# Schatten2021/rust-raytracing

Measured on AMD Instinct MI355X. Metric: Mrays/s (primary rays, whole node), 10k-sphere 1080p 64spp, higher is better.
Workload: dtype f64; 1 GPU; C2: 10k random spheres (scene seed 1), 1920x1080, 64 spp; width=1920, height=1080, rays_per_pixel=64, n_objects=10000, partition=single GPU

## Files before the change

### rust-raytracing_amd/__init__.py

```python
import ctypes as C
import math

import numpy as np

from . import abi
from .abi import (RTX_TUNE_NO_TILES, RTX_TUNE_NO_QNODES, RTX_TUNE_NO_PACKETS, RTX_TUNE_WF_PURE, RTX_TUNE_ONE_STAGE,
                  RTX_TUNE_TWO_STAGE, RTX_TUNE_BVH_MEDIAN, RTX_TUNE_TRI_LEAF_SHIFT, RTX_TUNE_THRESH_SHIFT, RTX_TUNE_PK_LDS_STACK, RTX_TUNE_NO_CUT, RTX_TUNE_INLINE_LEAVES, RTX_TUNE_HALVES, RTX_TUNE_NO_HALVES, RTX_TUNE_NO_TILE_LISTS)
from .abi import (OBJECT_DTYPE, RTX_KERNEL_WAVEFRONT, RTX_KERNEL_AUTO, RTX_KERNEL_BVH, RTX_KERNEL_EXACT, RTX_KERNEL_MIXED, RTX_KERNEL_MIXED_VERIFY, RTX_KERNEL_BVH_REGROUP,
                  RTX_PLANE, RTX_SPHERE, RTX_TRIANGLE, RtxError, load_library, RAY_DTYPE, HIT_DTYPE, FEATURE_DTYPE)

__all__ = ["LabKernel", "Vector3", "Material", "Sphere", "Plane", "Triangle", "Object", "Config", "Camera", "Scene",
           "SceneHandle", "RtxError", "device_count", "pack_objects", "OBJECT_DTYPE",
           "RTX_KERNEL_AUTO", "RTX_KERNEL_EXACT", "RTX_KERNEL_MIXED", "RTX_KERNEL_MIXED_VERIFY", "RTX_KERNEL_BVH", "RTX_KERNEL_BVH_REGROUP", "RTX_KERNEL_WAVEFRONT", "debug_host_scene",
           "RAY_DTYPE", "HIT_DTYPE", "FEATURE_DTYPE", "make_rays"]


class Vector3:
    __slots__ = ("x", "y", "z")

    def __init__(self, x=0.0, y=0.0, z=0.0):
        self.x, self.y, self.z = float(x), float(y), float(z)

    @staticmethod
    def zeros():
# ... 338 lines not shown
        sc = _scene_c(self.config, self.camera, packed)
        lib = load_library(self.config.wants_lab())
        abi.check(lib.rtx_any_hits(C.byref(sc), rays.ctypes.data, lim.ctypes.data if lim is not None else None, len(rays),
                                   occ.ctypes.data), lib)
        return occ.astype(bool)

    def multi_hits(self, origins, directions, k, t_max=None):
        rays = make_rays(origins, directions)
        n, k = len(rays), int(k)
        lim = _limits(t_max, n)
        hits = np.zeros((n, max(k, 0)), dtype=HIT_DTYPE)
        counts = np.zeros(n, dtype=np.uint32)
        packed = self.packed()
        sc = _scene_c(self.config, self.camera, packed)
        lib = load_library(self.config.wants_lab())
        abi.check(lib.rtx_multi_hits(C.byref(sc), rays.ctypes.data, lim.ctypes.data if lim is not None else None, n, k, hits.ctypes.data,
                                     counts.ctypes.data), lib)
        return _split_hits(hits) + (counts,)

    def trace_paths(self, origins, directions, ids=None):
        rays = make_rays(origins, directions)
        n = len(rays)
        pid = _path_ids(ids, n)
        rgb = np.zeros((n, 3), dtype=np.float64)
        seg = np.zeros(n, dtype=np.uint32)
        packed = self.packed()
        sc = _scene_c(self.config, self.camera, packed)
        lib = load_library(self.config.wants_lab())
        abi.check(lib.rtx_trace_paths(C.byref(sc), rays.ctypes.data, pid.ctypes.data if pid is not None else None, n, rgb.ctypes.data,
                                      seg.ctypes.data), lib)
        return rgb, seg


    def features(self, width, height):
        width, height = int(width), int(height)
        out = np.zeros((height, width), dtype=FEATURE_DTYPE)
        packed = self.packed()
        sc = _scene_c(self.config, self.camera, packed)
        lib = load_library(self.config.wants_lab())
        abi.check(lib.rtx_pixel_features(C.byref(sc), width, height, out.ctypes.data), lib)
        return _split_features(out)


TILE_LIST_WALK = 0xFFFFFFFF


class SceneHandle:

    def __init__(self, scene, device=0, lab=None):
        self.lab = scene.config.wants_lab() if lab is None else bool(lab)
        self._lib = load_library(self.lab)
        self.device = int(device)
        self.rays_per_pixel = int(scene.config.rays_per_pixel)
        self._h = C.c_void_p()
        packed = scene.packed()
        sc = _scene_c(scene.config, scene.camera, packed)
        self._check(self._lib.rtx_scene_upload(C.byref(sc), self.device, C.byref(self._h)))
        self._n_objects = len(packed)

    def _check(self, status):
        abi.check(status, self._lib)

    def set_config(self, config):
        if config.wants_lab() and not self.lab:
            raise ValueError("this handle lives in the product library; a lab config needs scene.upload(lab=True)")
        c = config.to_c()
        self._check(self._lib.rtx_scene_set_config(self._h, C.byref(c)))
        self.rays_per_pixel = int(config.rays_per_pixel)

    def set_scratch_limit(self, n_bytes):
        self._check(self._lib.rtx_scene_set_scratch_limit(self._h, int(n_bytes)))

    def set_camera(self, camera):
        c = camera.to_c()
        self._check(self._lib.rtx_scene_set_camera(self._h, C.byref(c)))

    def append_objects(self, packed):
        arr = packed if isinstance(packed, np.ndarray) else pack_objects(packed)
        arr = np.ascontiguousarray(arr, dtype=OBJECT_DTYPE)
        self._check(self._lib.rtx_scene_append_objects(self._h, arr.ctypes.data, len(arr)))
        self._n_objects += len(arr)

    def update_objects(self, indices, packed, mode="auto", stream=None):
        arr = packed if isinstance(packed, np.ndarray) else pack_objects(packed)
        arr = np.ascontiguousarray(arr, dtype=OBJECT_DTYPE)
        idx = np.ascontiguousarray(np.asarray(indices, dtype=np.uint64).reshape(-1))
        if len(idx) != len(arr):
            raise ValueError("update_objects: %d indices for %d objects" % (len(idx), len(arr)))
        how = C.c_uint32(0)
        self._check(self._lib.rtx_scene_update_objects(self._h, idx.ctypes.data, arr.ctypes.data, len(arr), _update_mode(mode),
                                                       C.c_void_p(int(stream)) if stream else None, C.byref(how)))
        return UPDATE_HOW[how.value]

    def set_visible(self, indices, visible, stream=None):
        idx = np.ascontiguousarray(np.asarray(indices, dtype=np.uint64).reshape(-1))
        how = C.c_uint32(0)
        self._check(self._lib.rtx_scene_set_visible(self._h, idx.ctypes.data if len(idx) else None, len(idx), int(visible),
                                                    C.c_void_p(int(stream)) if stream else None, C.byref(how)))
        return UPDATE_HOW[how.value]

    def hide(self, indices):
        return self.set_visible(indices, False)

    def show(self, indices):
        return self.set_visible(indices, True)

    def visible(self):
        mask = np.zeros(self._n_objects, dtype=np.uint8)
        self._check(self._lib.rtx_scene_get_visible(self._h, mask.ctypes.data if len(mask) else None))
        return mask.astype(bool)

    def debug_resident_digests(self):
        digests = (C.c_uint64 * 8)()
        self._check(self._lib.rtx_debug_resident_digests(self._h, digests))
        return tuple(int(v) for v in digests)

    def debug_resident_mesh_digests(self):
        digests = (C.c_uint64 * 16)()
        self._check(self._lib.rtx_debug_resident_mesh_digests(self._h, digests))
        return tuple(int(v) for v in digests)

    def debug_paths(self, width, height, row, max_steps):
        spp = self.rays_per_pixel
        steps = np.zeros((int(width), spp, int(max_steps)), dtype=PATH_STEP_DTYPE)
        counts = np.zeros((int(width), spp), dtype=np.uint32)
        self._check(self._lib.rtx_debug_paths(self._h, int(width), int(height), int(row), int(max_steps), steps.ctypes.data, counts.ctypes.data))
        return steps, counts

    def debug_path_bounds(self, origins, directions, objects, best_up, form=0, path_steps=0, want_records=False):
        rays = make_rays(origins, directions)
        n = len(rays)
        obj = np.ascontiguousarray(np.broadcast_to(np.asarray(objects, dtype=np.uint32), (n,)))
        bu = np.ascontiguousarray(np.broadcast_to(np.asarray(best_up, dtype=np.float32), (n,)))
        out = np.zeros((n, 8), dtype=np.uint32)
        extra = bool(want_records) or int(path_steps) > 0
        info = np.zeros(16, dtype=np.float64)
        rec = np.zeros((n, 16), dtype=np.uint32)
        path = np.zeros((n, int(path_steps), 16), dtype=np.uint32)
        self._check(self._lib.rtx_debug_path_bounds(self._h, rays.ctypes.data, obj.ctypes.data, bu.ctypes.data, n, int(form), out.ctypes.data,
                                                    info.ctypes.data if extra else None, rec.ctypes.data if extra else None,
                                                    path.ctypes.data if int(path_steps) > 0 else None, int(path_steps)))
        return (out, info, rec, path) if extra else out

    def debug_tile_lists(self):
        info = np.zeros(8, dtype=np.uint32)
        self._check(self._lib.rtx_debug_tile_lists(self._h, info.ctypes.data, None, None, 0))
        form, tiles_x, n_tiles, cap = (int(v) for v in info[:4])
        count = np.zeros(n_tiles, dtype=np.uint32)
        ent = np.zeros((n_tiles, cap, 12), dtype=np.uint32)
        if form and n_tiles:
            self._check(self._lib.rtx_debug_tile_lists(self._h, info.ctypes.data, count.ctypes.data, ent.ctypes.data, n_tiles))
        obj = ent[:, :, 9].astype(np.int64)
        obj[obj == 0xFFFFFFFF] = -1
        return {"form": form, "tiles_x": tiles_x, "n_tiles": n_tiles, "cap": cap, "count": count, "raw": ent[:, :, :8].copy(),
                "t_lb": np.ascontiguousarray(ent[:, :, 8]).view(np.float32), "object": obj, "is_record": ent[:, :, 10] == 1}

    def debug_sweep_filter(self, origins, directions, objects=None):
        rays = make_rays(origins, directions)
        n = len(rays)
        info = np.zeros(16, dtype=np.float64)
        obj = None if objects is None else np.ascontiguousarray(np.broadcast_to(np.asarray(objects, dtype=np.uint32), (n,)))
        out = np.zeros((n, 4 if obj is None else 24), dtype=np.uint32)
        self._check(self._lib.rtx_debug_sweep_filter(self._h, rays.ctypes.data if n else None, None if obj is None or not n else obj.ctypes.data,
                                                     n, out.ctypes.data if n else None, info.ctypes.data))
        return out, info

    def render_rows(self, width, height, row_begin, row_stride, n_rows, d_out_ptr, stream=None, want_stats=True):
        stats = abi.RtxStats()
        self._check(self._lib.rtx_render_rows(self._h, int(width), int(height), int(row_begin), int(row_stride),
                                            int(n_rows), C.c_void_p(int(d_out_ptr)),
                                            C.c_void_p(int(stream)) if stream else None,
                                            C.byref(stats) if want_stats else None))
        return stats if want_stats else None

    def render_blocks(self, width, height, block_rows, part, n_parts, d_out_ptr, stream=None, want_stats=True):
        stats = abi.RtxStats()
        self._check(self._lib.rtx_render_blocks(self._h, int(width), int(height), int(block_rows), int(part), int(n_parts),
                                              C.c_void_p(int(d_out_ptr)), C.c_void_p(int(stream)) if stream else None,
                                              C.byref(stats) if want_stats else None))
        return stats if want_stats else None

    def render_accumulate(self, width, height, sample_begin, n_samples, d_sum_ptr, d_sum_sq_ptr=None, block_rows=8, part=0, n_parts=1,
                          stream=None, want_stats=True):
        stats = abi.RtxStats()
        self._check(self._lib.rtx_render_blocks_accumulate(self._h, int(width), int(height), int(block_rows), int(part), int(n_parts),
                                                           int(sample_begin), int(n_samples), C.c_void_p(int(d_sum_ptr)) if d_sum_ptr else None,
                                                           C.c_void_p(int(d_sum_sq_ptr)) if d_sum_sq_ptr else None,
                                                           C.c_void_p(int(stream)) if stream else None, C.byref(stats) if want_stats else None))
        return stats if want_stats else None

    def render_refine(self, width, height, sample_begin, n_more, max_samples, threshold, floor, d_sum_ptr, d_sum_sq_ptr, d_extra_ptr, rounds=1,
                      block_rows=8, part=0, n_parts=1, stream=None, want_stats=True, want_result=True):
        stats = abi.RtxStats()
        result = (C.c_uint64 * 3)()
        self._check(self._lib.rtx_render_blocks_refine(self._h, int(width), int(height), int(block_rows), int(part), int(n_parts),
                                                       int(sample_begin), int(n_more), int(max_samples), int(rounds), float(threshold), float(floor),
                                                       C.c_void_p(int(d_sum_ptr)) if d_sum_ptr else None,
                                                       C.c_void_p(int(d_sum_sq_ptr)) if d_sum_sq_ptr else None,
                                                       C.c_void_p(int(d_extra_ptr)) if d_extra_ptr else None,
                                                       result if want_result else None,
                                                       C.c_void_p(int(stream)) if stream else None, C.byref(stats) if want_stats else None))
        return (tuple(int(v) for v in result) if want_result else None), (stats if want_stats else None)

    def trace_samples(self, width, height, d_ids_ptr, n, d_rgb_ptr, d_segments_ptr=None, stream=None, want_stats=True):
        stats = abi.RtxStats()
        self._check(self._lib.rtx_scene_trace_samples(self._h, int(width), int(height), C.c_void_p(int(d_ids_ptr)) if d_ids_ptr else None, int(n),
                                                      C.c_void_p(int(d_rgb_ptr)) if d_rgb_ptr else None,
                                                      C.c_void_p(int(d_segments_ptr)) if d_segments_ptr else None,
                                                      C.c_void_p(int(stream)) if stream else None, C.byref(stats) if want_stats else None))
        return stats if want_stats else None

    def progressive(self, width, height, moments=True):
        return Progressive(self, width, height, moments)

    def closest_hits(self, d_rays_ptr, n, d_hits_ptr, stream=None, want_stats=True):
        stats = abi.RtxStats()
        self._check(self._lib.rtx_scene_closest_hits(self._h, C.c_void_p(int(d_rays_ptr)), int(n), C.c_void_p(int(d_hits_ptr)),
                                                     C.c_void_p(int(stream)) if stream else None, C.byref(stats) if want_stats else None))
        return stats if want_stats else None

    def primary_hits(self, width, height, d_hits_ptr, stream=None, want_stats=True):
        stats = abi.RtxStats()
        self._check(self._lib.rtx_scene_primary_hits(self._h, int(width), int(height), C.c_void_p(int(d_hits_ptr)),
                                                     C.c_void_p(int(stream)) if stream else None, C.byref(stats) if want_stats else None))
        return stats if want_stats else None

    def any_hits(self, d_rays_ptr, d_t_max_ptr, n, d_out_ptr, stream=None, want_stats=True):
        stats = abi.RtxStats()
        self._check(self._lib.rtx_scene_any_hits(self._h, C.c_void_p(int(d_rays_ptr)),
                                                 C.c_void_p(int(d_t_max_ptr)) if d_t_max_ptr else None, int(n), C.c_void_p(int(d_out_ptr)),
                                                 C.c_void_p(int(stream)) if stream else None, C.byref(stats) if want_stats else None))
        return stats if want_stats else None

    def occluded(self, origins, directions, t_max=None):
        import torch
        rays = make_rays(origins, directions)
        n = len(rays)
        lim = _limits(t_max, n)
        dev = torch.device("cuda", self.device)
        d_rays = torch.from_numpy(rays.view(np.uint8)).to(dev)
        d_lim = torch.from_numpy(lim).to(dev) if lim is not None and n else None
        d_out = torch.empty(max(n, 1), dtype=torch.uint8, device=dev)
        torch.cuda.synchronize(dev)
        self.any_hits(d_rays.data_ptr(), d_lim.data_ptr() if d_lim is not None else None, n, d_out.data_ptr(), want_stats=True)
        return d_out[:n].cpu().numpy().astype(bool)

    def multi_hits(self, d_rays_ptr, d_t_max_ptr, n, k, d_hits_ptr, d_counts_ptr=None, stream=None, want_stats=True):
        stats = abi.RtxStats()
        self._check(self._lib.rtx_scene_multi_hits(self._h, C.c_void_p(int(d_rays_ptr)) if d_rays_ptr else None,
                                                   C.c_void_p(int(d_t_max_ptr)) if d_t_max_ptr else None, int(n), int(k),
                                                   C.c_void_p(int(d_hits_ptr)) if d_hits_ptr else None,
                                                   C.c_void_p(int(d_counts_ptr)) if d_counts_ptr else None,
                                                   C.c_void_p(int(stream)) if stream else None, C.byref(stats) if want_stats else None))
        return stats if want_stats else None

    def primary_multi_hits(self, width, height, k, d_hits_ptr, d_counts_ptr=None, stream=None, want_stats=True):
        stats = abi.RtxStats()
        self._check(self._lib.rtx_scene_primary_multi_hits(self._h, int(width), int(height), int(k),
                                                           C.c_void_p(int(d_hits_ptr)) if d_hits_ptr else None,
                                                           C.c_void_p(int(d_counts_ptr)) if d_counts_ptr else None,
                                                           C.c_void_p(int(stream)) if stream else None, C.byref(stats) if want_stats else None))
        return stats if want_stats else None

    def query_all(self, origins, directions, k, t_max=None):
        import torch
        rays = make_rays(origins, directions)
        n, k = len(rays), int(k)
        lim = _limits(t_max, n)
        dev = torch.device("cuda", self.device)
        d_rays = torch.from_numpy(rays.view(np.uint8)).to(dev)
        d_lim = torch.from_numpy(lim).to(dev) if lim is not None and n else None
        d_hits = torch.empty(max(n * k, 1) * HIT_DTYPE.itemsize, dtype=torch.uint8, device=dev)
        d_counts = torch.zeros(max(n, 1), dtype=torch.int32, device=dev)
        torch.cuda.synchronize(dev)
        self.multi_hits(d_rays.data_ptr(), d_lim.data_ptr() if d_lim is not None else None, n, k, d_hits.data_ptr(), d_counts.data_ptr(),
                        want_stats=True)
        hits = d_hits[:n * k * HIT_DTYPE.itemsize].cpu().numpy().view(HIT_DTYPE).reshape(n, k)
        return _split_hits(hits) + (d_counts[:n].cpu().numpy().view(np.uint32),)

    def pick_through(self, width, height, k):
        import torch
        width, height, k = int(width), int(height), int(k)
        n = width * height
        dev = torch.device("cuda", self.device)
        d_hits = torch.empty(max(n * k, 1) * HIT_DTYPE.itemsize, dtype=torch.uint8, device=dev)
        d_counts = torch.zeros(max(n, 1), dtype=torch.int32, device=dev)
        torch.cuda.synchronize(dev)
        self.primary_multi_hits(width, height, k, d_hits.data_ptr(), d_counts.data_ptr(), want_stats=True)
        hits = d_hits[:n * k * HIT_DTYPE.itemsize].cpu().numpy().view(HIT_DTYPE).reshape(height, width, k)
        return _split_hits(hits) + (d_counts[:n].cpu().numpy().view(np.uint32).reshape(height, width),)

    def trace_paths(self, d_rays_ptr, d_ids_ptr, n, d_rgb_ptr, d_segments_ptr=None, stream=None, want_stats=True):
        stats = abi.RtxStats()
        self._check(self._lib.rtx_scene_trace_paths(self._h, C.c_void_p(int(d_rays_ptr)), C.c_void_p(int(d_ids_ptr)) if d_ids_ptr else None,
                                                    int(n), C.c_void_p(int(d_rgb_ptr)),
                                                    C.c_void_p(int(d_segments_ptr)) if d_segments_ptr else None,
                                                    C.c_void_p(int(stream)) if stream else None, C.byref(stats) if want_stats else None))
        return stats if want_stats else None

    def radiance(self, origins, directions, ids=None, samples=1):
        import torch
        rays = make_rays(origins, directions)
        n, samples = len(rays), int(samples)
        if samples < 1:
            raise ValueError("samples >= 1")
        if samples == 1:
            pid = _path_ids(ids, n)
# ... 371 lines not shown
```

### rust-raytracing_amd/build.py

```python
import hashlib
import os
import shutil
import subprocess
from concurrent.futures import ThreadPoolExecutor

HERE = os.path.dirname(os.path.abspath(__file__))
CSRC = os.path.join(HERE, "csrc")
LIB = os.path.join(HERE, "librtx_hip.so")
LAB_LIB = os.path.join(HERE, "librtx_hip_lab.so")
OBJ_DIR = os.path.join(HERE, "build")
SOURCES = ["rtx_kernels.hip", "rtx_bvh_spheres.hip", "rtx_bvh_mesh.hip", "rtx_wavefront.hip", "rtx_query.hip", "rtx_update.hip", "rtx_pack.hip",
           "rtx_api.hip", "rtx_api_update.hip", "rtx_api_debug.hip"]
HEADERS = ["rtx_math.h", "rtx_scene.h", "rtx_bvh.h", "rtx_device.h", "rtx_traverse.h", "rtx_mesh_step.h", "rtx_wavefront.h",
           "rtx_launch.h", "rtx_refit.h", "rtx_pack.h", "rtx_host.h", "rtx_spk_units.h"]
FLAGS = ["--offload-arch=gfx950", "-O3", "-std=c++17", "-fPIC", "-ffp-contract=off",
         "-fno-fast-math", "-Wall", "-Wno-unused-function"]
LAB_FLAGS = ["-DRTX_LAB"]


def hipcc():
    exe = shutil.which("hipcc") or "/opt/rocm/bin/hipcc"
    if not os.path.exists(exe):
        raise RuntimeError("hipcc not found: librtx_hip.so cannot be built (there is no CPU fallback)")
    return exe


def _input_files():
    files = [os.path.join(CSRC, f) for f in HEADERS]
    files.append(os.path.join(HERE, "..", "include", "rtx_hip.h"))
    return files


def _digest(source, flags):
    h = hashlib.sha256()
    h.update(" ".join(flags).encode())
    for f in [os.path.join(CSRC, source)] + _input_files():
        with open(f, "rb") as fh:
            h.update(fh.read())
    return h.hexdigest()[:20]


def build(force=False, extra_flags=(), verbose=False, lib=None, jobs=None, lab=False):
    if lib is None:
        lib = LAB_LIB if lab else LIB
    flags = FLAGS + (LAB_FLAGS if lab else []) + list(extra_flags)
    os.makedirs(OBJ_DIR, exist_ok=True)
    exe = hipcc()
    objs, todo = [], []
    for s in SOURCES:
        obj = os.path.join(OBJ_DIR, "%s.%s.o" % (s[:-4], _digest(s, flags)))
        objs.append(obj)
        if force or not os.path.exists(obj):
            todo.append((s, obj))

    def compile_one(job):
        s, obj = job
        cmd = [exe] + flags + ["-c", os.path.join(CSRC, s), "-o", obj + ".tmp"]
        if verbose:
            print(" ".join(cmd), flush=True)
        subprocess.check_call(cmd)
        os.replace(obj + ".tmp", obj)

    if todo:
        with ThreadPoolExecutor(max_workers=jobs or min(len(todo), max(1, (os.cpu_count() or 2) - 1))) as ex:
            list(ex.map(compile_one, todo))
    stamp = lib + ".objs"
    want = "\n".join(os.path.basename(o) for o in objs) + "\n"
    have = open(stamp).read() if os.path.exists(stamp) else None
    if todo or not os.path.exists(lib) or have != want:
        if os.path.exists(stamp):
            os.remove(stamp)
        cmd = [exe, "--offload-arch=gfx950", "-shared", "-fPIC", "-Wl,-Bsymbolic"] + objs + ["-o", lib + ".tmp"]
        if verbose:
            print(" ".join(cmd), flush=True)
        subprocess.check_call(cmd)
        os.replace(lib + ".tmp", lib)
        with open(stamp, "w") as fh:
            fh.write(want)
    if not extra_flags:
        keep = set()
        for st in os.listdir(HERE):
            if st.endswith(".so.objs") and os.path.exists(os.path.join(HERE, st[:-5])):
                keep.update(open(os.path.join(HERE, st)).read().split())
        for f in os.listdir(OBJ_DIR):
            if f.endswith(".o") and f not in keep:
                os.remove(os.path.join(OBJ_DIR, f))
    return lib


def build_all(force=False, verbose=False):
    return build(force=force, verbose=verbose), build(force=force, verbose=verbose, lab=True)


if __name__ == "__main__":
    import sys
    for path in build_all(force="--force" in sys.argv, verbose=True):
        print(path)
```

### rust-raytracing_amd/csrc/rtx_api.hip

```cpp
#include "rtx_host.h"

#include <cmath>
#include <cstdio>
#include <cstdlib>
#include <cstring>
#include <string>
#include <thread>
#include <vector>

namespace {

bool device_is_gfx950(int dev)
{
    hipDeviceProp_t prop;
    if (hipGetDeviceProperties(&prop, dev) != hipSuccess) return false;
    return std::strncmp(prop.gcnArchName, "gfx950", 6) == 0;
}

constexpr size_t kDefaultScratchBytes = (size_t)24576 << 20;

}

#ifndef RTX_GRABS_PER_WAVE
#define RTX_GRABS_PER_WAVE 16
#endif

constexpr uint64_t kHalvesBelowRays = 0;

constexpr size_t kWorkWords = kQueryRefineWords;

namespace {

template <class T>
int32_t upload_vec(RtxSceneHandle_ *h, const std::vector<T> &v, const T **out)
{
    *out = nullptr;
    if (v.empty()) return RTX_OK;
    void *d = nullptr;
    RTX_HIP_CHECK(hipMalloc(&d, v.size() * sizeof(T)));
    h->scene_allocs.push_back(d);
    RTX_HIP_CHECK(hipMemcpy(d, v.data(), v.size() * sizeof(T), hipMemcpyHostToDevice));
    *out = static_cast<const T *>(d);
    return RTX_OK;
}

void apply_config(RtxSceneHandle_ *h, const RtxConfig &cfg)
{
    h->cfg = cfg;
    h->sv.rays_per_pixel = cfg.rays_per_pixel;
    h->sv.max_bounces = cfg.max_bounces;
    h->sv.focal_length = cfg.focal_length;
    h->sv.focal_offset = cfg.focal_offset;
    h->sv.non_focal_offset = cfg.non_focal_offset;
    h->sv.seed = cfg.seed;
    h->sv.tuning = cfg.tuning;
    h->sv_dirty = true;
}

#ifdef RTX_LAB
constexpr bool kLabBuild = true;
#else
constexpr bool kLabBuild = false;
#endif

int32_t check_config(const RtxConfig &cfg)
{
    if (cfg.kernel > RTX_KERNEL_WAVEFRONT) return fail(RTX_ERR_INVALID_ARGUMENT, "RtxConfig.kernel: unknown kernel id");
    if (cfg.tuning & ~(uint32_t)RTX_TUNE_KNOWN_MASK)
        return fail(RTX_ERR_UNSUPPORTED, "RtxConfig.tuning: a bit include/rtx_hip.h does not name");
    if (!kLabBuild && (cfg.tuning & (uint32_t)RTX_TUNE_LAB_MASK))
        return fail(RTX_ERR_UNSUPPORTED, "RtxConfig.tuning: a RTX_TUNE_LAB_MASK bit selects a kernel that exists in librtx_hip_lab.so only "
                                         "(this is the product library)");
    if (cfg.max_bounces == UINT64_MAX)
        return fail(RTX_ERR_INVALID_ARGUMENT, "RtxConfig.max_bounces + 1 overflows");
    if (cfg.rays_per_pixel > 0xFFFFFFFFull) return fail(RTX_ERR_INVALID_ARGUMENT, "RtxConfig.rays_per_pixel exceeds 2^32-1");
    return RTX_OK;
}

int32_t grow(void **p, size_t *have, size_t want)
{
    if (*have >= want && *p) return RTX_OK;
    if (*p) { RTX_HIP_CHECK(hipFree(*p)); *p = nullptr; *have = 0; }
    if (want == 0) return RTX_OK;
    RTX_HIP_CHECK(hipMalloc(p, want));
    *have = want;
    return RTX_OK;
}

}

RTX_HOST_BEGIN

int usable_device_count()
{
    int n = 0;
    if (hipGetDeviceCount(&n) != hipSuccess) { (void)hipGetLastError(); return 0; }
    int ok = 0;
    for (int d = 0; d < n; ++d) ok += device_is_gfx950(d) ? 1 : 0;
    return ok;
}

void drop_update_tables(RtxSceneHandle_ *h)
{
    auto &b = h->upd;
    for (void *q : { (void *)b.levels, (void *)b.box32, (void *)b.reach, (void *)b.all_levels, (void *)b.tribox32, (void *)b.tri_reach, (void *)b.keep })
        if (q) (void)hipFree(q);
    b.keep = nullptr; b.keep_valid = false;
    b.levels = nullptr; b.box32 = nullptr; b.reach = nullptr; b.valid = false;
    b.all_levels = nullptr; b.tribox32 = nullptr; b.tri_reach = nullptr; b.mesh_valid = false;
}

int32_t upload_packed(RtxSceneHandle_ *h, const PackedScene &p)
{
    const SceneView sv_before = h->sv;
    std::vector<void *> old_allocs;
    old_allocs.swap(h->scene_allocs);
    {
        SceneView sv = p.sv;
        sv.rays_per_pixel = h->sv.rays_per_pixel; sv.max_bounces = h->sv.max_bounces;
        sv.focal_length = h->sv.focal_length; sv.focal_offset = h->sv.focal_offset; sv.non_focal_offset = h->sv.non_focal_offset;
        sv.seed = h->sv.seed; sv.tuning = h->sv.tuning;
        h->sv = sv;
    }
    h->sv.cam_pos = mk(h->cam.position[0], h->cam.position[1], h->cam.position[2]);
    h->sv.to_world_x = mk(h->cam.to_world_space[0], h->cam.to_world_space[1], h->cam.to_world_space[2]);
    h->sv.to_world_y = mk(h->cam.to_world_space[3], h->cam.to_world_space[4], h->cam.to_world_space[5]);
    h->sv.to_world_z = mk(h->cam.to_world_space[6], h->cam.to_world_space[7], h->cam.to_world_space[8]);

    int32_t rc = RTX_OK;
    if (!rc) rc = upload_vec(h, p.bvh4.nodes, &h->sv.bvh_nodes);
    if (!rc) rc = upload_vec(h, p.qnodes, &h->sv.bvh_qnodes);
    if (!rc) rc = upload_vec(h, p.q3nodes, &h->sv.bvh_q3nodes);
    if (!rc) rc = upload_vec(h, p.bvh.prims, &h->sv.bvh_prims);
    if (!rc) rc = upload_vec(h, p.leaf32, &h->sv.bvh_leaf_f32);
    if (!rc) rc = upload_vec(h, p.leaf_cr, &h->sv.bvh_leaf_cr);
    if (!rc) rc = upload_vec(h, p.spheres, &h->sv.spheres);
    if (!rc) rc = upload_vec(h, p.sphere_id, &h->sv.sphere_id);
    if (!rc) rc = upload_vec(h, p.planes, &h->sv.planes);
    if (!rc) rc = upload_vec(h, p.tris, &h->sv.tris);
    if (!rc) rc = upload_vec(h, p.mats, &h->sv.materials);
    if (!rc) rc = upload_vec(h, p.sph32, &h->sv.sphere_f32);
    if (!rc) rc = upload_vec(h, p.tri32, &h->sv.tri_f32);
    if (!rc) rc = upload_vec(h, p.tri_fidx, &h->sv.tri_fidx);
    if (!rc) rc = upload_vec(h, p.tri_geo, &h->sv.tri_geo);
    if (rc) {
        for (void *d : h->scene_allocs) (void)hipFree(d);
        h->scene_allocs.swap(old_allocs);
        h->sv = sv_before;
        return rc;
    }
    for (void *d : old_allocs) (void)hipFree(d);
    h->sv_dirty = true;
    h->refit = make_refit_tables(p);
    drop_update_tables(h);
    return RTX_OK;
}

int32_t check_watchdog(RtxSceneHandle_ *h, bool wait)
{
    if (!h->watchdog_pending) return RTX_OK;
    if (wait) RTX_HIP_CHECK(hipEventSynchronize(h->ev_watchdog));
    else {
        const hipError_t q = hipEventQuery(h->ev_watchdog);
        if (q == hipErrorNotReady) return RTX_OK;
        RTX_HIP_CHECK(q);
    }
    h->watchdog_pending = false;
    if ((h->h_watchdog[0] | h->h_watchdog[1]) != 0ull) {
        const unsigned long long n = h->h_watchdog[0] + h->h_watchdog[1];
        h->h_watchdog[0] = h->h_watchdog[1] = 0ull;
        return fail(RTX_ERR_HIP, "an earlier render on this scene raised its watchdog word (internal error: the sweep kernel's round "
                                 "bound, or a full survivors' queue): " + std::to_string(n) + " event(s); its image is incomplete");
    }
    return RTX_OK;
}

int32_t adopt_stream(RtxSceneHandle_ *h, hipStream_t stream)
{
    if (h->have_last_stream && h->last_stream != stream && h->have_done) RTX_HIP_CHECK(hipStreamWaitEvent(stream, h->ev_done, 0));
    h->last_stream = stream;
    h->have_last_stream = true;
    return RTX_OK;
}

RTX_HOST_END

namespace {

void free_handle(RtxSceneHandle_ *h)
{
    if (!h) return;
    (void)hipSetDevice(h->device);
    for (void *p : h->scene_allocs) (void)hipFree(p);
    drop_update_tables(h);
    if (h->upd.h_entries) (void)hipHostFree(h->upd.h_entries);
    if (h->upd.d_entries) (void)hipFree(h->upd.d_entries);
    if (h->upd.d_status) (void)hipFree(h->upd.d_status);
    if (h->upd.h_status) (void)hipHostFree(h->upd.h_status);
    if (h->samples) (void)hipFree(h->samples);
    if (h->acc) (void)hipFree(h->acc);
    if (h->tables) (void)hipFree(h->tables);
    if (h->h_tables) (void)hipHostFree(h->h_tables);
    if (h->state) (void)hipFree(h->state);
    if (h->wf_state) (void)hipFree(h->wf_state);
    if (h->tile_lists) (void)hipFree(h->tile_lists);
    if (h->counters) (void)hipFree(h->counters);
    if (h->counters_stage1) (void)hipFree(h->counters_stage1);
    if (h->work_counter) (void)hipFree(h->work_counter);
    if (h->d_sv) (void)hipFree(h->d_sv);
    if (h->d_rv) (void)hipFree(h->d_rv);
    {
        auto &b = h->half2;
        if (b.stream) { (void)hipStreamSynchronize(b.stream); (void)hipStreamDestroy(b.stream); }
        for (hipEvent_t e : { b.fork, b.join, b.stage1_done }) if (e) (void)hipEventDestroy(e);
        for (void *q : { (void *)b.counters, (void *)b.counters_stage1, (void *)b.work_counter, (void *)b.d_rv, (void *)b.state, b.queue })
            if (q) (void)hipFree(q);
    }
    if (h->h_watchdog) (void)hipHostFree(h->h_watchdog);
    if (h->ev_watchdog) (void)hipEventDestroy(h->ev_watchdog);
    if (h->ev_done) (void)hipEventDestroy(h->ev_done);
    for (auto &e : h->ev) if (e) (void)hipEventDestroy(e);
    delete h;
}

int32_t check_scene_args(const RtxScene *scene, const char *who)
{
    if (!scene) return fail(RTX_ERR_INVALID_ARGUMENT, std::string(who) + ": null scene");
    if (scene->n_objects && !scene->objects) return fail(RTX_ERR_INVALID_ARGUMENT, std::string(who) + ": objects is null");
    if (scene->n_objects > 0xFFFFFFF0ull) return fail(RTX_ERR_INVALID_ARGUMENT, std::string(who) + ": too many objects");
    return check_config(scene->config);
}

int32_t check_device(int32_t device, const char *who)
{
    int n_dev = 0;
    if (hipGetDeviceCount(&n_dev) != hipSuccess || n_dev == 0) {
        (void)hipGetLastError();
        return fail(RTX_ERR_NO_DEVICE, "no HIP device visible; librtx_hip has no CPU fallback");
    }
    if (device < 0 || device >= n_dev) return fail(RTX_ERR_INVALID_ARGUMENT, std::string(who) + ": bad device index");
    if (!device_is_gfx950(device)) return fail(RTX_ERR_NO_DEVICE, "device is not gfx950 (MI355X); this library targets gfx950 only");
    return RTX_OK;
}

int32_t create_handle(const RtxScene *scene, const PackedScene &p, int32_t device, RtxSceneHandle_ **out)
{
    *out = nullptr;
    RTX_HIP_CHECK(hipSetDevice(device));
    RtxSceneHandle_ *h = new RtxSceneHandle_();
    h->device = device;
    hipDeviceProp_t prop;
    if (hipGetDeviceProperties(&prop, device) != hipSuccess) { free_handle(h); return fail(RTX_ERR_HIP, "hipGetDeviceProperties failed"); }
    h->n_cus = prop.multiProcessorCount;
    h->cam = scene->camera;
    apply_config(h, scene->config);
    if (int32_t irc = upload_packed(h, p)) { free_handle(h); return irc; }
    h->objects.assign(scene->objects, scene->objects + scene->n_objects);

    hipError_t e = hipMalloc((void **)&h->counters, sizeof(Counters) * kCounterShards);
    if (e == hipSuccess) e = hipMalloc((void **)&h->counters_stage1, sizeof(Counters) * kCounterShards);
    if (e == hipSuccess) e = hipMalloc((void **)&h->work_counter, kWorkWords * sizeof(unsigned long long));
    if (e == hipSuccess) e = hipMalloc((void **)&h->d_sv, sizeof(SceneView));
    if (e == hipSuccess) e = hipMalloc((void **)&h->d_rv, sizeof(RowsView));
    if (e == hipSuccess) e = hipHostMalloc((void **)&h->h_watchdog, 2 * sizeof(unsigned long long), hipHostMallocDefault);
    if (e == hipSuccess) { h->h_watchdog[0] = h->h_watchdog[1] = 0ull; e = hipEventCreateWithFlags(&h->ev_watchdog, hipEventDisableTiming); }
    if (e == hipSuccess) e = hipEventCreateWithFlags(&h->ev_done, hipEventDisableTiming);
    for (int k = 0; k < 4 && e == hipSuccess; ++k) e = hipEventCreate(&h->ev[k]);
    if (e != hipSuccess) { free_handle(h); return fail(RTX_ERR_HIP, std::string("scene scratch: ") + hipGetErrorString(e)); }
    *out = h;
    return RTX_OK;
}

size_t scratch_cap(const RtxSceneHandle_ *h, size_t mine_bytes)
{
    size_t cap_bytes = h->scratch_limit ? h->scratch_limit : kDefaultScratchBytes;
    size_t free_b = 0, total_b = 0;
    if (hipMemGetInfo(&free_b, &total_b) == hipSuccess) {
        const size_t avail = (free_b + mine_bytes) / 4 * 3;
        if (cap_bytes > avail) cap_bytes = avail;
    } else (void)hipGetLastError();
    return cap_bytes;
}

struct CounterSums {
    unsigned long long segments = 0, exact = 0, filter = 0, box = 0, mismatches = 0, watchdog = 0;
    void operator+=(const CounterSums &o) { segments += o.segments; exact += o.exact; filter += o.filter; box += o.box; mismatches += o.mismatches; watchdog += o.watchdog; }
    void operator-=(const CounterSums &o) { segments -= o.segments; exact -= o.exact; filter -= o.filter; box -= o.box; mismatches -= o.mismatches; watchdog -= o.watchdog; }
};

CounterSums sum_counters(const Counters (&c)[kCounterShards])
{
    CounterSums s;
    for (int k = 0; k < kCounterShards; ++k) {
        s.segments += c[k].segments; s.exact += c[k].exact_tests; s.filter += c[k].filter_tests;
        if (k >= 2) s.box += c[k].pad_;
    }
    s.mismatches = c[0].pad_; s.watchdog = c[1].pad_;
    return s;
}

int32_t read_counters(const Counters *d_counters, CounterSums &sums)
{
    Counters host[kCounterShards];
    RTX_HIP_CHECK(hipMemcpy(host, d_counters, sizeof host, hipMemcpyDeviceToHost));
    sums = sum_counters(host);
    return RTX_OK;
}

RowsView rows_view(const RtxSceneHandle_ *h, uint32_t width, uint32_t height, uint32_t row_begin, uint32_t row_stride,
                   uint32_t row_block, uint32_t n_rows, uint32_t tiles_x, uint32_t per_sample)
{
    RowsView rv{};
    rv.width = width; rv.height = height;
    rv.row_begin = row_begin; rv.row_stride = row_stride; rv.n_rows = n_rows; rv.row_block = row_block;
    rv.npix = n_rows * width;
    rv.tiles_x = tiles_x;
    rv.div_width = make_fastdiv(width); rv.div_row_block = make_fastdiv(row_block); rv.div_npix = make_fastdiv(rv.npix);
    rv.div_tiles_x = make_fastdiv(tiles_x); rv.div_per_sample = make_fastdiv(per_sample);
    rv.sin_x = h->tables; rv.cos_x = h->tables + width;
    rv.sin_y = h->tables + 2 * (size_t)width; rv.cos_y = rv.sin_y + n_rows;
    return rv;
}

uint32_t grab_size(uint64_t n_rays, int n_cus, uint32_t grabs_per_wave)
{
    const uint64_t per_wave = n_rays / ((uint64_t)n_cus * 16u * grabs_per_wave);
    return (uint32_t)(per_wave >= 512 ? 512 : (per_wave <= 64 ? 64 : (per_wave & ~(uint64_t)63)));
}

int32_t begin_launches(RtxSceneHandle_ *h, hipStream_t stream)
{
    if (h->sv_dirty) {
        RTX_HIP_CHECK(hipMemcpyAsync(h->d_sv, &h->sv, sizeof(SceneView), hipMemcpyHostToDevice, stream));
        h->sv_dirty = false;
    }
    RTX_HIP_CHECK(hipMemsetAsync(h->counters, 0, sizeof(Counters) * kCounterShards, stream));
    return RTX_OK;
}

struct Range { const void *base; size_t bytes; };
bool ranges_overlap(const Range *r, int n)
{
    for (int i = 0; i < n; ++i)
        for (int j = i + 1; j < n; ++j) {
            const uintptr_t a = (uintptr_t)r[i].base, b = (uintptr_t)r[j].base;
            if (a && b && a < b + r[j].bytes && b < a + r[i].bytes) return true;
        }
    return false;
}

}

extern "C" {

int32_t rtx_version(void) { return RTX_HIP_VERSION; }

const char *rtx_last_error(void) { return last_error().c_str(); }

int32_t rtx_device_count(void) { return usable_device_count(); }

int32_t rtx_lab_build(void) { return kLabBuild ? 1 : 0; }

int32_t rtx_camera_new(const double position[3], const double direction[3], double fov, RtxCamera *out)
{
    if (!position || !direction || !out) return fail(RTX_ERR_INVALID_ARGUMENT, "rtx_camera_new: null argument");
    V3 cam_forward = vnorm(mk(direction[0], direction[1], direction[2]));
    V3 cam_right = cross(cam_forward, mk(0., 0., -1.));
    V3 cam_up = cross(cam_forward, cam_right);
    V3 rx = mk(cam_right.x, cam_up.x, cam_forward.x);
    V3 ry = mk(cam_right.y, cam_up.y, cam_forward.y);
    V3 rz = mk(cam_right.z, cam_up.z, cam_forward.z);
    double a = rx.x, b = rx.y, c = rx.z, d = ry.x, e = ry.y, f = ry.z, g = rz.x, hh = rz.y, i = rz.z;
    double sum1 = a * e * i, sum2 = b * f * g, sum3 = c * d * hh;
    double sub1 = g * e * c, sub2 = hh * f * a, sub3 = i * d * b;
    double det = (sum1 + sum2 + sum3) - (sub1 + sub2 + sub3);
    V3 ax = mk(e * i - f * hh, c * hh - b * i, b * f - c * e);
    V3 ay = mk(f * g - d * i, a * i - c * g, c * d - a * f);
    V3 az = mk(d * hh - e * g, b * g - a * hh, a * e - b * d);
    V3 ix = vdivs(ax, det), iy = vdivs(ay, det), iz = vdivs(az, det);
    out->fov = fov;
    for (int k = 0; k < 3; ++k) { out->position[k] = position[k]; out->direction[k] = direction[k]; }
    const V3 w[3] = { rx, ry, rz }, cinv[3] = { ix, iy, iz };
    for (int r = 0; r < 3; ++r) {
        out->to_world_space[3 * r] = w[r].x; out->to_world_space[3 * r + 1] = w[r].y; out->to_world_space[3 * r + 2] = w[r].z;
        out->to_cam_space[3 * r] = cinv[r].x; out->to_cam_space[3 * r + 1] = cinv[r].y; out->to_cam_space[3 * r + 2] = cinv[r].z;
    }
    return RTX_OK;
}

int32_t rtx_scene_upload(const RtxScene *scene, int32_t device, RtxSceneHandle *out)
{
    if (!scene || !out) return fail(RTX_ERR_INVALID_ARGUMENT, "rtx_scene_upload: null argument");
    *out = nullptr;
    if (int32_t rc = check_scene_args(scene, "rtx_scene_upload")) return rc;
    if (int32_t rc = check_device(device, "rtx_scene_upload")) return rc;
    PackedScene p;
    if (int32_t rc = pack_scene(scene, p)) return rc;
    return create_handle(scene, p, device, out);
}

int32_t rtx_scene_free(RtxSceneHandle scene)
{
    if (!scene) return RTX_OK;
    (void)hipSetDevice(scene->device);
    const int32_t rc = check_watchdog(scene, true);
    free_handle(scene);
    return rc;
}

int32_t rtx_scene_set_config(RtxSceneHandle scene, const RtxConfig *config)
{
    if (!scene || !config) return fail(RTX_ERR_INVALID_ARGUMENT, "rtx_scene_set_config: null argument");
    if (int32_t rc = check_config(*config)) return rc;
    if (int32_t rc = check_watchdog(scene, false)) return rc;
    apply_config(scene, *config);
    return RTX_OK;
}

int32_t rtx_scene_set_scratch_limit(RtxSceneHandle scene, uint64_t bytes)
{
    if (!scene) return fail(RTX_ERR_INVALID_ARGUMENT, "rtx_scene_set_scratch_limit: null scene");
    scene->scratch_limit = (size_t)bytes;
    return RTX_OK;
}

int32_t rtx_scene_set_camera(RtxSceneHandle scene, const RtxCamera *camera)
{
    if (!scene || !camera) return fail(RTX_ERR_INVALID_ARGUMENT, "rtx_scene_set_camera: null argument");
    if (int32_t rc = check_watchdog(scene, false)) return rc;
    scene->cam = *camera;
    scene->sv.cam_pos = mk(camera->position[0], camera->position[1], camera->position[2]);
    scene->sv.to_world_x = mk(camera->to_world_space[0], camera->to_world_space[1], camera->to_world_space[2]);
    scene->sv.to_world_y = mk(camera->to_world_space[3], camera->to_world_space[4], camera->to_world_space[5]);
    scene->sv.to_world_z = mk(camera->to_world_space[6], camera->to_world_space[7], camera->to_world_space[8]);
    scene->sv_dirty = true;
    return RTX_OK;
}

}

static uint32_t blocks_row_count(uint32_t height, uint32_t block, uint32_t part, uint32_t n_parts)
{
    if (block == 0 || n_parts == 0 || part >= n_parts) return 0;
    const uint64_t n_blocks = ((uint64_t)height + block - 1) / block;
    if (part >= n_blocks) return 0;
    const uint64_t mine = (n_blocks - part + n_parts - 1) / n_parts;
    uint64_t rows = mine * block;
    const uint64_t last = part + (mine - 1) * (uint64_t)n_parts;
    if (last == n_blocks - 1) rows -= n_blocks * block - height;
    return (uint32_t)rows;
}

static int32_t ensure_tables(RtxSceneHandle_ *h, uint32_t width, uint32_t height, uint32_t row_begin, uint32_t row_stride,
                             uint32_t row_block, uint32_t n_rows, hipStream_t stream)
{
    const size_t tdbl = 2 * (size_t)width + 2 * (size_t)n_rows;
    const bool t_same = h->t_valid && h->t_w == width && h->t_h == height && h->t_rb == row_begin &&
                        h->t_rs == row_stride && h->t_blk == row_block && h->t_nr == n_rows && h->t_fov == h->cam.fov;
    if (!t_same) {
        if (h->have_done) RTX_HIP_CHECK(hipEventSynchronize(h->ev_done));
        if (h->h_tables_doubles < tdbl) {
            if (h->h_tables) RTX_HIP_CHECK(hipHostFree(h->h_tables));
            h->h_tables = nullptr; h->h_tables_doubles = 0;
            RTX_HIP_CHECK(hipHostMalloc((void **)&h->h_tables, tdbl * sizeof(double), hipHostMallocDefault));
            h->h_tables_doubles = tdbl;
        }
        {
            size_t have = h->tables_doubles * sizeof(double);
            if (int32_t rc = grow((void **)&h->tables, &have, tdbl * sizeof(double))) return rc;
            h->tables_doubles = have / sizeof(double);
        }
        const double fov = h->cam.fov;
        const double vertical_fov = (double)height / (double)width * fov;
        double *sx = h->h_tables, *cx = sx + width, *sy = cx + width, *cy = sy + n_rows;
        for (uint32_t x = 0; x < width; ++x) {
            double u = (double)x / (double)width;
            double angle_x = fov * (u - 0.5);
            ::sincos(angle_x, &sx[x], &cx[x]);
        }
        for (uint32_t k = 0; k < n_rows; ++k) {
            const uint32_t kb = k / row_block;
            double v = (double)(row_begin + kb * row_stride + (k - kb * row_block)) / (double)height;
            double angle_y = vertical_fov * (v - 0.5);
            ::sincos(angle_y, &sy[k], &cy[k]);
        }
        RTX_HIP_CHECK(hipMemcpyAsync(h->tables, h->h_tables, tdbl * sizeof(double), hipMemcpyHostToDevice, stream));
        h->t_w = width; h->t_h = height; h->t_rb = row_begin; h->t_rs = row_stride; h->t_blk = row_block; h->t_nr = n_rows;
        h->t_fov = fov; h->t_valid = true;
    }
    return RTX_OK;
}

namespace {

struct BandPlan {
    uint32_t kernel = RTX_KERNEL_AUTO;
    bool tiled = false; uint32_t tiles_x = 0;
    uint64_t per_sample64 = 0, batch = 0;
    uint64_t tile_list_bytes = 0;
    bool spheres_kernel = false, mesh_kernel = false, spheres_two_stage = false;
    bool halves = false;
};
struct BandRun { float trace_ms = 0.f, resolve_ms = 0.f, stage1_ms = 0.f; CounterSums stage1; uint32_t launches = 0; };

uint32_t choose_kernel(const SceneView &sv, const RtxConfig &cfg, uint32_t npix, uint64_t spp)
{
    const uint64_t outside_tree = ((sv.bvh_flags & 1u) ? 0u : sv.n_spheres) + (uint64_t)(sv.n_tri_filter - sv.n_tri_tree);
    uint32_t kernel = cfg.kernel;
    const bool want_tiles = (cfg.tuning & RTX_TUNE_NO_TILES) == 0u;
    if (kernel == RTX_KERNEL_AUTO) {
        if (sv.n_bvh_nodes != 0 && outside_tree <= 64) {
            const bool mesh = (sv.bvh_flags & 2u) != 0u && sv.n_tri_tree >= 1024u;
            kernel = mesh ? RTX_KERNEL_BVH_REGROUP : RTX_KERNEL_BVH;
            if (mesh && (uint64_t)npix * spp >= (1ull << 20) && want_tiles && wavefront_mesh_supported(sv, true))
                kernel = RTX_KERNEL_WAVEFRONT;
        } else {
            kernel = RTX_KERNEL_MIXED;
        }
    }

    if (kernel == RTX_KERNEL_BVH || kernel == RTX_KERNEL_BVH_REGROUP || kernel == RTX_KERNEL_WAVEFRONT) {
        const bool sphere_tree = sv.n_bvh_nodes != 0 && (sv.bvh_flags & 19u) == 17u;
        const bool tri_tree = sv.n_bvh_nodes != 0 && (sv.bvh_flags & 2u) != 0u;
        if (sphere_tree) kernel = RTX_KERNEL_BVH;
        else if (!tri_tree) kernel = RTX_KERNEL_MIXED;
        else if (kernel == RTX_KERNEL_BVH) kernel = RTX_KERNEL_BVH_REGROUP;
    }
    if (kernel == RTX_KERNEL_WAVEFRONT && !wavefront_mesh_supported(sv, want_tiles)) kernel = RTX_KERNEL_BVH_REGROUP;
    return kernel;
}

int32_t plan_batch(const RtxSceneHandle_ *h, BandPlan &plan, uint32_t width, uint32_t n_rows, uint64_t spp)
{
    const uint32_t kernel = plan.kernel, tuning = h->cfg.tuning;
    const bool want_tiles = (tuning & RTX_TUNE_NO_TILES) == 0u;
    plan.tiled = (kernel == RTX_KERNEL_BVH || kernel == RTX_KERNEL_BVH_REGROUP || kernel == RTX_KERNEL_WAVEFRONT) && want_tiles;
    plan.tiles_x = plan.tiled ? (width + 7u) / 8u : 0u;
    const uint64_t per_sample64 = plan.tiled ? (uint64_t)plan.tiles_x * ((n_rows + 7u) / 8u) * 64u : (uint64_t)n_rows * width;
    if (per_sample64 > 0xFFFFFFF0ull) return fail(RTX_ERR_INVALID_ARGUMENT, "rtx_render_rows: more than 2^32 ray slots per sample");
    plan.per_sample64 = per_sample64;
    plan.batch = spp;
    const bool sph2 = kernel == RTX_KERNEL_BVH && (h->sv.bvh_flags & 2u) == 0u && h->sv.n_bvh_nodes != 0;
    const uint64_t per_ray = 4 * sizeof(double) + (kernel == RTX_KERNEL_WAVEFRONT ? wavefront_state_bytes(1u << 20, 1) >> 20 : 0) +
                             (sph2 ? 64 + 5 : 0);
    const size_t cap_bytes = scratch_cap(h, h->samples_bytes + h->wf_bytes + h->tile_lists_bytes);
    if ((tuning & RTX_TUNE_NO_TILE_LISTS) == 0u && plan.tiled) {
        if (sph2) plan.tile_list_bytes = bvh_spheres_tile_list_bytes(per_sample64);
        else if (kernel == RTX_KERNEL_WAVEFRONT) plan.tile_list_bytes = wavefront_tile_list_bytes(per_sample64);
        if (plan.tile_list_bytes > cap_bytes / 4) plan.tile_list_bytes = 0;
    }
    const uint64_t fixed = plan.tile_list_bytes +
                           (sph2 ? (uint64_t)bvh_spheres_queue_bytes(0, h->n_cus) + bvh_spheres_spill_bytes(h->sv, h->n_cus) : 0) +
                           (kernel == RTX_KERNEL_WAVEFRONT ? (uint64_t)wavefront_state_bytes(0, 1) + wavefront_spill_bytes(h->sv, h->n_cus) : 0) +
                           (kernel == RTX_KERNEL_MIXED || kernel == RTX_KERNEL_MIXED_VERIFY ? (uint64_t)mixed_state_bytes(h->n_cus) : 0);
    const uint64_t room = cap_bytes > fixed ? cap_bytes - fixed : 0;
    const uint64_t fit = room * 8 / (per_sample64 * (per_ray * 8 + 1));
    const uint64_t fit32 = 0xFFFFFFF0ull / per_sample64;
    if (plan.batch > fit) plan.batch = fit ? fit : 1;
    if (plan.batch > fit32) plan.batch = fit32;
    return RTX_OK;
}

void plan_forms(const RtxSceneHandle_ *h, BandPlan &plan, uint64_t spp, bool may_halve)
{
    const SceneView &sv = h->sv;
    const uint32_t kernel = plan.kernel, tuning = h->cfg.tuning;
    plan.spheres_kernel = kernel == RTX_KERNEL_BVH && (sv.bvh_flags & 2u) == 0u && sv.n_bvh_nodes != 0;
    plan.mesh_kernel = kernel == RTX_KERNEL_BVH_REGROUP && (sv.bvh_flags & 2u) != 0u;
    plan.spheres_two_stage = plan.spheres_kernel && h->cfg.max_bounces > 0 && (tuning & RTX_TUNE_ONE_STAGE) == 0u &&
                             (plan.batch * plan.per_sample64 >= (1ull << 20) || (tuning & RTX_TUNE_TWO_STAGE) != 0u) &&
                             bvh_spheres_two_stage_ok(sv, plan.tiled);
    const bool halves_can = may_halve && plan.spheres_two_stage && plan.batch == spp && spp >= 2;
    plan.halves = halves_can && (tuning & RTX_TUNE_NO_HALVES) == 0u &&
                  ((tuning & RTX_TUNE_HALVES) != 0u || plan.per_sample64 * spp <= kHalvesBelowRays);
}

int32_t grow_scratch(RtxSceneHandle_ *h, const BandPlan &plan, uint32_t npix, uint64_t spp, bool own_acc)
{
    const uint32_t kernel = plan.kernel;
    const uint64_t batch_rays = plan.batch * plan.per_sample64;
    if (spp > 0)
        if (int32_t rc = grow((void **)&h->samples, &h->samples_bytes,
                              (size_t)(batch_rays * 4 * sizeof(double)) + nonzero_mask_bytes(batch_rays))) return rc;
    if (own_acc && plan.batch < spp)
        if (int32_t rc = grow((void **)&h->acc, &h->acc_bytes, (size_t)npix * 3 * sizeof(double))) return rc;
    if (kernel == RTX_KERNEL_BVH || kernel == RTX_KERNEL_BVH_REGROUP) {
        if (!plan.spheres_kernel && !plan.mesh_kernel) return fail(RTX_ERR_HIP, "internal: no tree kernel for this scene");
        const size_t need = plan.spheres_kernel ? bvh_spheres_spill_bytes(h->sv, h->n_cus) : bvh_mesh_spill_bytes(h->sv, h->n_cus);
        if (int32_t rc = grow((void **)&h->state, &h->state_bytes, need)) return rc;
    }
    if (kernel == RTX_KERNEL_MIXED || kernel == RTX_KERNEL_MIXED_VERIFY)
        if (int32_t rc = grow((void **)&h->state, &h->state_bytes, mixed_state_bytes(h->n_cus))) return rc;
    if (plan.spheres_two_stage) {
        if (int32_t rc = grow(&h->wf_state, &h->wf_bytes, bvh_spheres_queue_bytes(batch_rays, h->n_cus))) return rc;
        if (plan.tile_list_bytes != 0)
            if (int32_t rc = grow(&h->tile_lists, &h->tile_lists_bytes, (size_t)plan.tile_list_bytes)) return rc;
    }
    if (kernel == RTX_KERNEL_WAVEFRONT) {
        if (int32_t rc = grow((void **)&h->state, &h->state_bytes, wavefront_spill_bytes(h->sv, h->n_cus))) return rc;
        if (int32_t rc = grow(&h->wf_state, &h->wf_bytes, wavefront_state_bytes(batch_rays, wavefront_levels(h->sv)))) return rc;
        if (plan.tile_list_bytes != 0)
            if (int32_t rc = grow(&h->tile_lists, &h->tile_lists_bytes, (size_t)plan.tile_list_bytes)) return rc;
    }
    return RTX_OK;
}

uint32_t sphere_flags(uint32_t tuning)
{
    return (tuning & RTX_TUNE_NO_PACKETS) ? 1u : 0u;
}

int32_t launch_halves(RtxSceneHandle_ *h, const BandPlan &plan, RowsView rv, double *d_out_rgb, hipStream_t stream, bool stats,
                      BandRun &run)
{
    const uint64_t spp = h->cfg.rays_per_pixel, per_sample64 = plan.per_sample64;
    auto &b = h->half2;
    if (!b.stream) {
        int least = 0, greatest = 0;
        RTX_HIP_CHECK(hipDeviceGetStreamPriorityRange(&least, &greatest));
        RTX_HIP_CHECK(hipStreamCreateWithPriority(&b.stream, hipStreamNonBlocking, least));
        RTX_HIP_CHECK(hipEventCreateWithFlags(&b.fork, hipEventDisableTiming));
        RTX_HIP_CHECK(hipEventCreateWithFlags(&b.join, hipEventDisableTiming));
        RTX_HIP_CHECK(hipEventCreate(&b.stage1_done));
        RTX_HIP_CHECK(hipMalloc((void **)&b.counters, sizeof(Counters) * kCounterShards));
        RTX_HIP_CHECK(hipMalloc((void **)&b.counters_stage1, sizeof(Counters) * kCounterShards));
        RTX_HIP_CHECK(hipMalloc((void **)&b.work_counter, sizeof(unsigned long long)));
        RTX_HIP_CHECK(hipMalloc((void **)&b.d_rv, sizeof(RowsView)));
    }
    const uint64_t ns[2] = { (spp + 1) / 2, spp / 2 };
    if (int32_t rc = grow((void **)&b.state, &b.state_bytes, bvh_spheres_spill_bytes(h->sv, h->n_cus))) return rc;
    if (int32_t rc = grow(&b.queue, &b.queue_bytes, bvh_spheres_queue_bytes(ns[1] * per_sample64, h->n_cus))) return rc;
    struct Join {
        RtxSceneHandle_ *h; hipStream_t main; bool forked = false;
        ~Join() {
            if (!forked) return;
            if (hipEventRecord(h->half2.join, h->half2.stream) != hipSuccess || hipStreamWaitEvent(main, h->half2.join, 0) != hipSuccess) {
                (void)hipGetLastError(); (void)hipStreamSynchronize(h->half2.stream);
            }
        }
    } join{h, stream};
    RTX_HIP_CHECK(hipMemsetAsync(b.counters, 0, sizeof(Counters) * kCounterShards, stream));
    RTX_HIP_CHECK(hipMemsetAsync(rv.nonzero, 0, nonzero_mask_bytes(per_sample64 * spp), stream));
    if (stats) RTX_HIP_CHECK(hipEventRecord(h->ev[0], stream));
    RTX_HIP_CHECK(hipEventRecord(b.fork, stream));
    RTX_HIP_CHECK(hipStreamWaitEvent(b.stream, b.fork, 0));
    join.forked = true;
    for (int k = 0; k < 2; ++k) {
        RowsView r = rv;
        r.sample_begin = k == 0 ? 0u : (uint32_t)ns[0];
        r.n_samples = (uint32_t)ns[k];
        r.n_rays = per_sample64 * ns[k];
        r.nonzero_base = k == 0 ? 0 : per_sample64 * ns[0];
        r.grab = grab_size(r.n_rays, h->n_cus, RTX_GRABS_PER_WAVE / 2);
        hipStream_t st = k == 0 ? stream : b.stream;
        RTX_HIP_CHECK(hipMemcpyAsync(k == 0 ? h->d_rv : b.d_rv, &r, sizeof(RowsView), hipMemcpyHostToDevice, st));
        RTX_HIP_CHECK(hipMemsetAsync(k == 0 ? h->work_counter : b.work_counter, 0, sizeof(unsigned long long), st));
        RTX_HIP_CHECK(launch_trace_bvh_spheres(h->d_sv, h->sv, k == 0 ? h->d_rv : b.d_rv, r,
                                               h->samples + (k == 0 ? 0 : (size_t)(per_sample64 * ns[0]) * 4), k == 0 ? h->counters : b.counters,
                                               k == 0 ? h->work_counter : b.work_counter, reinterpret_cast<uint32_t *>(k == 0 ? h->state : b.state),
                                               h->n_cus, k == 0 ? h->wf_state : b.queue, sphere_flags(h->cfg.tuning), st,
                                               stats ? (k == 0 ? h->counters_stage1 : b.counters_stage1) : nullptr,
                                               stats ? (k == 0 ? h->ev[3] : b.stage1_done) : nullptr,
                                               nullptr, false));
    }
    RTX_HIP_CHECK(hipEventRecord(b.join, b.stream));
    RTX_HIP_CHECK(hipStreamWaitEvent(stream, b.join, 0));
    join.forked = false;
    run.launches = 1;
    if (stats) RTX_HIP_CHECK(hipEventRecord(h->ev[1], stream));
    rv.sample_begin = 0; rv.n_samples = (uint32_t)spp; rv.n_rays = per_sample64 * spp;
    RTX_HIP_CHECK(launch_resolve(h->samples, h->acc, d_out_rgb, rv, (uint32_t)per_sample64, spp, true, true, stream));
    if (stats) {
        RTX_HIP_CHECK(hipEventRecord(h->ev[2], stream));
        RTX_HIP_CHECK(hipEventSynchronize(h->ev[2]));
        RTX_HIP_CHECK(hipEventElapsedTime(&run.trace_ms, h->ev[0], h->ev[1]));
        RTX_HIP_CHECK(hipEventElapsedTime(&run.resolve_ms, h->ev[1], h->ev[2]));
        float c0 = 0.f, c1 = 0.f;
        RTX_HIP_CHECK(hipEventElapsedTime(&c0, h->ev[0], h->ev[3]));
        RTX_HIP_CHECK(hipEventElapsedTime(&c1, h->ev[0], b.stage1_done));
        run.stage1_ms = c0 > c1 ? c0 : c1;
        for (const Counters *snap : { h->counters_stage1, b.counters_stage1 }) {
            CounterSums s1;
            if (int32_t rc = read_counters(snap, s1)) return rc;
            run.stage1 += s1;
        }
    }
    return RTX_OK;
}

int32_t launch_batch(RtxSceneHandle_ *h, const BandPlan &plan, const RowsView &rv, bool first_batch, hipStream_t stream, bool stats)
{
    const uint32_t kernel = plan.kernel, tuning = h->cfg.tuning;
    uint32_t *const state = reinterpret_cast<uint32_t *>(h->state);
    if (kernel != RTX_KERNEL_EXACT && kernel != RTX_KERNEL_WAVEFRONT)
        RTX_HIP_CHECK(hipMemsetAsync(h->work_counter, 0, sizeof(unsigned long long), stream));
    if (kernel == RTX_KERNEL_EXACT) {
        RTX_HIP_CHECK(launch_trace_exact(h->d_sv, h->d_rv, rv, h->samples, h->counters, stream));
#ifdef RTX_LAB
        if (h->transcript)
            RTX_HIP_CHECK(launch_trace_transcript(h->d_sv, h->d_rv, rv, h->transcript, h->transcript_counts, h->transcript_steps, stream));
#endif
    } else if (kernel == RTX_KERNEL_WAVEFRONT) {
        RTX_HIP_CHECK(launch_trace_wavefront(h->d_sv, h->sv, h->d_rv, rv, h->samples, h->wf_state, h->counters, state, h->n_cus, stream,
                                             plan.tile_list_bytes != 0 ? h->tile_lists : nullptr, first_batch));
    } else if (kernel == RTX_KERNEL_BVH_REGROUP) {
        RTX_HIP_CHECK(launch_trace_bvh_mesh(h->d_sv, h->sv, h->d_rv, rv, h->samples, h->counters, h->work_counter, state, h->n_cus, stream));
    } else if (kernel == RTX_KERNEL_BVH) {
        const bool two = plan.spheres_two_stage;
        RTX_HIP_CHECK(launch_trace_bvh_spheres(h->d_sv, h->sv, h->d_rv, rv, h->samples, h->counters, h->work_counter, state, h->n_cus,
                                               two ? h->wf_state : nullptr, sphere_flags(tuning), stream,
                                               stats && two ? h->counters_stage1 : nullptr, stats && two ? h->ev[3] : nullptr,
                                               two && plan.tile_list_bytes != 0 ? h->tile_lists : nullptr, first_batch));
    } else {
        RTX_HIP_CHECK(launch_trace_mixed(h->d_sv, h->sv, h->d_rv, rv, h->samples, h->state, h->counters, h->work_counter, h->n_cus,
                                         kernel == RTX_KERNEL_MIXED_VERIFY, stream));
    }
    return RTX_OK;
}

int32_t launch_batches(RtxSceneHandle_ *h, const BandPlan &plan, RowsView rv, const SampleRange &sr, double *d_out_rgb, hipStream_t stream,
                       bool stats, BandRun &run)
{
    const uint64_t spp = sr.n;
    const bool accumulate = sr.sum != nullptr;
    CounterSums before;
    for (uint64_t s0 = 0; s0 < spp; s0 += plan.batch) {
        const uint64_t ns = (spp - s0 < plan.batch) ? spp - s0 : plan.batch;
        rv.sample_begin = (uint32_t)(sr.begin + s0); rv.n_samples = (uint32_t)ns;
        rv.n_rays = plan.per_sample64 * ns;
        rv.grab = grab_size(rv.n_rays, h->n_cus, RTX_GRABS_PER_WAVE);
        RTX_HIP_CHECK(hipMemcpyAsync(h->d_rv, &rv, sizeof(RowsView), hipMemcpyHostToDevice, stream));
        RTX_HIP_CHECK(hipMemsetAsync(rv.nonzero, 0, nonzero_mask_bytes(rv.n_rays), stream));
        if (stats) RTX_HIP_CHECK(hipEventRecord(h->ev[0], stream));
        if (int32_t rc = launch_batch(h, plan, rv, s0 == 0, stream, stats)) return rc;
        ++run.launches;
        if (stats) RTX_HIP_CHECK(hipEventRecord(h->ev[1], stream));
        if (accumulate)
            RTX_HIP_CHECK(launch_resolve(h->samples, sr.sum, nullptr, rv, (uint32_t)plan.per_sample64, spp, false, false, stream, sr.sum_sq));
        else
            RTX_HIP_CHECK(launch_resolve(h->samples, h->acc, d_out_rgb, rv, (uint32_t)plan.per_sample64, spp, s0 == 0, s0 + ns == spp, stream));
        if (!stats) continue;
        RTX_HIP_CHECK(hipEventRecord(h->ev[2], stream));
        RTX_HIP_CHECK(hipEventSynchronize(h->ev[2]));
        float a = 0.f, b = 0.f;
        RTX_HIP_CHECK(hipEventElapsedTime(&a, h->ev[0], h->ev[1]));
        RTX_HIP_CHECK(hipEventElapsedTime(&b, h->ev[1], h->ev[2]));
        run.trace_ms += a; run.resolve_ms += b;
        if (plan.spheres_two_stage) {
            float c = 0.f;
            RTX_HIP_CHECK(hipEventElapsedTime(&c, h->ev[0], h->ev[3]));
            run.stage1_ms += c;
            CounterSums snapshot, now;
            if (int32_t rc = read_counters(h->counters_stage1, snapshot)) return rc;
            if (int32_t rc = read_counters(h->counters, now)) return rc;
            run.stage1 += snapshot; run.stage1 -= before;
            before = now;
        }
    }
    return RTX_OK;
}

int32_t finish_stats(RtxSceneHandle_ *h, const BandPlan &plan, const BandRun &run, uint64_t primary_rays, hipStream_t stream, RtxStats *stats)
{
    if (plan.kernel == RTX_KERNEL_MIXED || plan.kernel == RTX_KERNEL_MIXED_VERIFY || plan.spheres_two_stage) {
        if (h->watchdog_pending) RTX_HIP_CHECK(hipEventSynchronize(h->ev_watchdog));
        if (int32_t rc = check_watchdog(h, false)) return rc;
        RTX_HIP_CHECK(hipMemcpyAsync(h->h_watchdog, &h->counters[1].pad_, sizeof(unsigned long long), hipMemcpyDeviceToHost, stream));
        if (plan.halves) RTX_HIP_CHECK(hipMemcpyAsync(h->h_watchdog + 1, &h->half2.counters[1].pad_, sizeof(unsigned long long), hipMemcpyDeviceToHost, stream));
        RTX_HIP_CHECK(hipEventRecord(h->ev_watchdog, stream));
        h->watchdog_pending = true;
    }
    if (!stats) return RTX_OK;
    RTX_HIP_CHECK(hipStreamSynchronize(stream));
    CounterSums c;
    if (int32_t rc = read_counters(h->counters, c)) return rc;
    if (plan.halves) {
        CounterSums more;
        if (int32_t rc = read_counters(h->half2.counters, more)) return rc;
        c += more;
    }
    stats->segments = c.segments; stats->exact_tests = c.exact; stats->filter_tests = c.filter; stats->box_tests = c.box;
    stats->filter_mismatches = c.mismatches;
    if (c.watchdog != 0) {
        h->watchdog_pending = false; h->h_watchdog[0] = h->h_watchdog[1] = 0ull;
        return fail(RTX_ERR_HIP, "trace kernel raised its watchdog word (internal error: round bound / full survivors' queue): " +
                                     std::to_string(c.watchdog) + " event(s)");
    }
    stats->primary_rays = primary_rays;
    stats->trace_ms = run.trace_ms; stats->resolve_ms = run.resolve_ms; stats->stage1_ms = run.stage1_ms;
    stats->trace_launches = run.launches;
    stats->kernel = plan.kernel;
    stats->stage1_box_tests = run.stage1.box; stats->stage1_filter_tests = run.stage1.filter; stats->stage1_exact_tests = run.stage1.exact;
    return RTX_OK;
}

}

RTX_HOST_BEGIN

int32_t render_band(RtxSceneHandle h, uint32_t width, uint32_t height, uint32_t row_begin, uint32_t row_stride,
                    uint32_t row_block, uint32_t n_rows, double *d_out_rgb, void *stream_, RtxStats *stats,
                    const SampleRange *accumulate)
{
    hipStream_t stream = static_cast<hipStream_t>(stream_);
    if (stats) std::memset(stats, 0, sizeof *stats);
    if (n_rows == 0 || width == 0) return RTX_OK;
    if (!accumulate && !d_out_rgb) return fail(RTX_ERR_INVALID_ARGUMENT, "rtx_render_rows: null output");
    if ((uint64_t)n_rows * width > 0xFFFFFFF0ull) return fail(RTX_ERR_INVALID_ARGUMENT, "rtx_render_rows: more than 2^32 pixels per call");
    if (accumulate) {
        if ((uint64_t)n_rows * width >= 0xFFFFFFF0ull)
            return fail(RTX_ERR_INVALID_ARGUMENT, "rtx_render_blocks_accumulate: 2^32 - 16 pixels per call or more");
        const size_t bytes = (size_t)n_rows * width * 3 * sizeof(double);
        const Range r[2] = { { accumulate->sum, bytes }, { accumulate->sum_sq, bytes } };
        if (ranges_overlap(r, 2)) return fail(RTX_ERR_INVALID_ARGUMENT, "rtx_render_blocks_accumulate: d_sum and d_sum_sq overlap");
    }
    RTX_HIP_CHECK(hipSetDevice(h->device));
    if (int32_t rc = check_watchdog(h, false)) return rc;
    if (int32_t rc = adopt_stream(h, stream)) return rc;
    DoneGuard done_guard{h, stream};

    const uint32_t npix = n_rows * width;
    SampleRange sr;
    if (accumulate) sr = *accumulate; else sr.n = h->cfg.rays_per_pixel;
    const uint64_t spp = sr.n;
    if (accumulate && h->sv.n_objects == 0) {
        if (stats) {
            RTX_HIP_CHECK(hipStreamSynchronize(stream));
            stats->primary_rays = (uint64_t)npix * spp;
            stats->kernel = h->cfg.kernel;
        }
        return RTX_OK;
    }
    if (h->sv.n_objects == 0 && spp > 0) {
        RTX_HIP_CHECK(hipMemsetAsync(d_out_rgb, 0, (size_t)npix * 3 * sizeof(double), stream));
        if (stats) {
            RTX_HIP_CHECK(hipStreamSynchronize(stream));
            stats->primary_rays = (uint64_t)npix * spp;
            stats->kernel = h->cfg.kernel;
        }
        return RTX_OK;
    }
    BandPlan plan;
    plan.kernel = choose_kernel(h->sv, h->cfg, npix, spp);
    if (int32_t rc = plan_batch(h, plan, width, n_rows, spp)) return rc;
    plan_forms(h, plan, spp, accumulate == nullptr);
#ifdef RTX_LAB
    h->tl_form = 0;
    if (plan.tile_list_bytes != 0 && spp > 0 && !plan.halves) {
        const bool no_packets = (h->cfg.tuning & RTX_TUNE_NO_PACKETS) != 0u;
        if (plan.kernel == RTX_KERNEL_WAVEFRONT) h->tl_form = (no_packets && (h->sv.bvh_flags & 4u) != 0u) ? 0u : 2u;
        else if (plan.kernel == RTX_KERNEL_BVH && plan.spheres_two_stage) h->tl_form = no_packets ? 0u : 1u;
    }
    h->tl_tiles_x = plan.tiles_x;
    h->tl_tiles = (uint32_t)(plan.per_sample64 >> 6);
#endif
    if (int32_t rc = ensure_tables(h, width, height, row_begin, row_stride, row_block, n_rows, stream)) return rc;
    if (int32_t rc = grow_scratch(h, plan, npix, spp, accumulate == nullptr)) return rc;

    RowsView rv = rows_view(h, width, height, row_begin, row_stride, row_block, n_rows, plan.tiles_x, (uint32_t)plan.per_sample64);
    rv.nonzero = spp > 0 ? reinterpret_cast<uint32_t *>(h->samples + (size_t)(plan.batch * plan.per_sample64) * 4) : nullptr;
    if (int32_t rc = begin_launches(h, stream)) return rc;
    BandRun run;
    if (spp == 0) {
        rv.n_samples = 0; rv.n_rays = 0; rv.tiles_x = 0;
        RTX_HIP_CHECK(launch_resolve(nullptr, nullptr, d_out_rgb, rv, npix, 0, true, true, stream));
    } else if (plan.halves) {
        if (int32_t rc = launch_halves(h, plan, rv, d_out_rgb, stream, stats != nullptr, run)) return rc;
    } else {
        if (int32_t rc = launch_batches(h, plan, rv, sr, d_out_rgb, stream, stats != nullptr, run)) return rc;
    }
    return finish_stats(h, plan, run, (uint64_t)npix * spp, stream, stats);
}

RTX_HOST_END

namespace {

struct QueryRequest {
    uint32_t mode = kQueryClosest;
    uint32_t width = 0, height = 0;
    uint32_t row_begin = 0, row_stride = 1, row_block = 1, n_rows = 0;
    uint64_t n = 0;
    const RtxRay *rays = nullptr;
    RtxHit *hits = nullptr;
    uint8_t *occluded = nullptr; const double *t_max = nullptr;
    double *rgb = nullptr;
    const uint64_t *ids = nullptr; uint32_t *segments = nullptr;
    RtxPixelFeatures *features = nullptr;
    double *sum = nullptr, *sum_sq = nullptr; uint32_t *extra = nullptr;
    double threshold = 0.0, floor = 0.0;
    uint32_t sample_begin = 0, n_more = 0, max_samples = 0, rounds = 0;
    uint64_t *result = nullptr;
    uint32_t k = 0; uint32_t *counts = nullptr;
};

}

static int32_t query_run(RtxSceneHandle_ *h, const QueryRequest &req, void *stream_, RtxStats *stats)
{
    hipStream_t stream = static_cast<hipStream_t>(stream_);
    const uint64_t n = req.n;
    const bool pick = req.width != 0;
    const bool refine = req.mode == kQueryRefine;
    if (stats) std::memset(stats, 0, sizeof *stats);
    if (req.result) req.result[0] = req.result[1] = req.result[2] = 0;
    if (n == 0) return RTX_OK;
    RTX_HIP_CHECK(hipSetDevice(h->device));
    if (int32_t rc = check_watchdog(h, false)) return rc;
    if (int32_t rc = adopt_stream(h, stream)) return rc;
    DoneGuard done_guard{h, stream};

    const bool walk = h->cfg.kernel != RTX_KERNEL_EXACT && query_tree_kind(h->sv) != 0u;
    if (req.mode == kQueryAnyHit && h->sv.n_objects == 0) {
        RTX_HIP_CHECK(hipMemsetAsync(req.occluded, 0, n, stream));
        if (stats) {
            RTX_HIP_CHECK(hipStreamSynchronize(stream));
            stats->segments = n;
            stats->kernel = RTX_KERNEL_EXACT;
        }
        return RTX_OK;
    }
    if (req.mode == kQueryPaths && h->sv.n_objects == 0) {
        RTX_HIP_CHECK(hipMemsetAsync(req.rgb, 0, n * 3 * sizeof(double), stream));
        if (req.segments) RTX_HIP_CHECK(hipMemsetAsync(req.segments, 0, n * sizeof(uint32_t), stream));
        if (stats) {
            RTX_HIP_CHECK(hipStreamSynchronize(stream));
            stats->primary_rays = n;
            stats->kernel = RTX_KERNEL_EXACT;
        }
        return RTX_OK;
    }
    if (refine && h->sv.n_objects == 0) {
        if (stats || req.result) RTX_HIP_CHECK(hipStreamSynchronize(stream));
        if (stats) stats->kernel = RTX_KERNEL_EXACT;
        return RTX_OK;
    }
    if (pick) {
        if (int32_t rc = ensure_tables(h, req.width, req.height, req.row_begin, req.row_stride, req.row_block, req.n_rows, stream)) return rc;
        RowsView rv = rows_view(h, req.width, req.height, req.row_begin, req.row_stride, req.row_block, req.n_rows, 0u, (uint32_t)n);
        rv.n_samples = 1; rv.n_rays = n;
        RTX_HIP_CHECK(hipMemcpyAsync(h->d_rv, &rv, sizeof(RowsView), hipMemcpyHostToDevice, stream));
    }
    uint32_t spill_entries = walk ? query_spill_entries(h->sv) : 0u;
    if (spill_entries != 0u) {
        const size_t cap_bytes = scratch_cap(h, h->state_bytes);
        const size_t per_entry = query_spill_bytes(1u, h->n_cus);
        if ((size_t)spill_entries * per_entry > cap_bytes) spill_entries = (uint32_t)(cap_bytes / per_entry);
        if (int32_t rc = grow((void **)&h->state, &h->state_bytes, query_spill_bytes(spill_entries, h->n_cus))) return rc;
    }
    if (int32_t rc = begin_launches(h, stream)) return rc;
    RTX_HIP_CHECK(hipMemsetAsync(h->work_counter, 0, (refine ? kQueryRefineRule : 1) * sizeof(unsigned long long), stream));
    if (refine) {
        const QueryRefineRule rule{ req.threshold, req.floor, req.sample_begin, req.n_more, req.max_samples, req.rounds };
        RTX_HIP_CHECK(hipMemcpyAsync(h->work_counter + kQueryRefineRule, &rule, sizeof rule, hipMemcpyHostToDevice, stream));
    }
    QueryArgs qa{};
    qa.rays = reinterpret_cast<const QueryRay *>(req.rays);
    qa.rv = pick ? h->d_rv : nullptr;
    qa.n = n; qa.mode = req.mode;
    if (req.mode == kQueryAnyHit) { qa.occluded = req.occluded; qa.t_max = req.t_max; }
    else if (req.mode == kQueryPaths) { qa.rgb = req.rgb; qa.ids = reinterpret_cast<const unsigned long long *>(req.ids); qa.segments = req.segments; }
    else if (req.mode == kQueryFeatures) qa.features = reinterpret_cast<QueryFeatures *>(req.features);
    else if (refine) {
        qa.sum = req.sum; qa.sum_sq = req.sum_sq; qa.extra = req.extra;
    }
    else if (req.mode == kQueryMulti) {
        qa.mode = kQueryMulti | (req.k << kQueryMultiShift);
        qa.hits = reinterpret_cast<QueryHit *>(req.hits); qa.t_max = req.t_max; qa.counts = req.counts;
    }
    else qa.hits = reinterpret_cast<QueryHit *>(req.hits);
    if (stats) RTX_HIP_CHECK(hipEventRecord(h->ev[0], stream));
    RTX_HIP_CHECK(launch_query_closest(h->d_sv, h->sv, qa, walk, spill_entries ? reinterpret_cast<uint32_t *>(h->state) : nullptr,
                                       spill_entries, h->n_cus, h->counters, h->work_counter, stream));
    uint64_t counts[3] = { 0, 0, 0 };
    if (refine && (stats || req.result)) {
        if (stats) RTX_HIP_CHECK(hipEventRecord(h->ev[1], stream));
        RTX_HIP_CHECK(hipStreamSynchronize(stream));
        RTX_HIP_CHECK(hipMemcpy(counts, h->work_counter + kQueryRefineCounts, sizeof counts, hipMemcpyDeviceToHost));
        if (req.result) std::memcpy(req.result, counts, sizeof counts);
    }
    if (stats) {
        if (!refine) RTX_HIP_CHECK(hipEventRecord(h->ev[1], stream));
        RTX_HIP_CHECK(hipEventSynchronize(h->ev[1]));
        float ms = 0.f;
        RTX_HIP_CHECK(hipEventElapsedTime(&ms, h->ev[0], h->ev[1]));
        CounterSums c;
        if (int32_t rc = read_counters(h->counters, c)) return rc;
        stats->segments = c.segments; stats->exact_tests = c.exact; stats->filter_tests = c.filter; stats->box_tests = c.box;
        if (refine) stats->primary_rays = counts[1];
        if (req.mode == kQueryPaths) stats->primary_rays = n;
        if (req.mode == kQueryFeatures) stats->primary_rays = n * h->cfg.rays_per_pixel;
        stats->trace_ms = ms;
        stats->trace_launches = 1;
        stats->kernel = walk ? RTX_KERNEL_BVH : RTX_KERNEL_EXACT;
    }
    return RTX_OK;
}

extern "C" {

int32_t rtx_render_rows(RtxSceneHandle h, uint32_t width, uint32_t height, uint32_t row_begin, uint32_t row_stride,
                        uint32_t n_rows, double *d_out_rgb, void *stream, RtxStats *stats)
{
    if (!h) return fail(RTX_ERR_INVALID_ARGUMENT, "rtx_render_rows: null scene");
    if (n_rows != 0 && width != 0) {
        if (row_stride == 0) return fail(RTX_ERR_INVALID_ARGUMENT, "rtx_render_rows: row_stride == 0");
        if ((uint64_t)row_begin + (uint64_t)(n_rows - 1) * row_stride >= height)
            return fail(RTX_ERR_INVALID_ARGUMENT, "rtx_render_rows: rows exceed the image height");
    }
    return render_band(h, width, height, row_begin, row_stride, 1u, n_rows, d_out_rgb, stream, stats);
}

uint32_t rtx_blocks_row_count(uint32_t height, uint32_t block_rows, uint32_t part, uint32_t n_parts)
{
    return blocks_row_count(height, block_rows, part, n_parts);
}

int32_t rtx_render_blocks(RtxSceneHandle h, uint32_t width, uint32_t height, uint32_t block_rows, uint32_t part, uint32_t n_parts,
                          double *d_out_rgb, void *stream, RtxStats *stats)
{
    if (!h) return fail(RTX_ERR_INVALID_ARGUMENT, "rtx_render_blocks: null scene");
    if (block_rows == 0 || n_parts == 0 || part >= n_parts) return fail(RTX_ERR_INVALID_ARGUMENT, "rtx_render_blocks: bad partition");
// ... 460 lines not shown
```

### rust-raytracing_amd/csrc/rtx_api_debug.hip

```cpp
#include "rtx_host.h"

#include <algorithm>
#include <cstring>

extern "C" {

int32_t rtx_debug_host_scene(const RtxScene *scene, uint64_t *stats)
{
    if (!scene || !stats) return fail(RTX_ERR_INVALID_ARGUMENT, "rtx_debug_host_scene: null argument");
    if (scene->n_objects && !scene->objects) return fail(RTX_ERR_INVALID_ARGUMENT, "rtx_debug_host_scene: objects is null");
    PackedScene p;
    if (int32_t rc = pack_scene(scene, p)) return rc;
    return check_packed(p, scene->objects, stats);
}

#ifdef RTX_LAB
static int32_t fetch_resident(RtxSceneHandle_ *h, bool mesh, PackedScene &p)
{
    RTX_HIP_CHECK(hipSetDevice(h->device));
    RTX_HIP_CHECK(hipDeviceSynchronize());
    const SceneView &sv = h->sv;
    auto fetch = [](auto &vec, const void *src, size_t count) -> hipError_t {
        vec.resize(count);
        return count && src ? hipMemcpy(vec.data(), src, count * sizeof(vec[0]), hipMemcpyDeviceToHost) : hipSuccess;
// ... 390 lines not shown
            Frame f = std::move(todo.back());
            todo.pop_back();
            const uint32_t idx = f.link & ~kBvhFlatNode;
            if (idx >= nodes.size() || ++visited > nodes.size() || f.path.size() / 2 >= stride)
                return fail(RTX_ERR_INVALID_ARGUMENT, "rtx_debug_path_bounds: the resident tree is not a tree of the recorded depth");
            const Bvh4Node &w = nodes[idx];
            for (uint32_t c = 0; c < 4; ++c) {
                uint32_t lnk, cnt;
                if (f.link & kBvhFlatNode) {
                    const float l4[4] = { w.b[0].x, w.b[0].y, w.b[0].z, w.b[0].w }, c4[4] = { w.b[1].x, w.b[1].y, w.b[1].z, w.b[1].w };
                    lnk = bits(l4[c]); cnt = bits(c4[c]);
                } else { lnk = bits(w.a[c].w); cnt = bits(w.b[c].w); }
                if (cnt == 0xFFFFFFFFu) continue;
                std::vector<uint32_t> path = f.path;
                path.push_back(f.link); path.push_back(c);
                if (cnt == 0u) { todo.push_back({lnk, std::move(path)}); continue; }
                const bool tri = (cnt & kBvhTriLeaf) != 0u;
                for (uint32_t k = 0; k < (cnt & 0xFFFFu); ++k) {
                    const size_t e = (size_t)lnk + k;
                    if (e >= (tri ? tri_fidx.size() : prims.size())) return fail(RTX_ERR_INVALID_ARGUMENT, "rtx_debug_path_bounds: a leaf entry outside its array");
                    const size_t row = tri ? prims.size() + e : e;
                    lens[row] = (uint32_t)(path.size() / 2);
                    std::copy(path.begin(), path.end(), steps.begin() + (ptrdiff_t)(2 * row * stride));
                }
            }
        }
    }
    std::vector<uint32_t> entries(n), rows(n);
    std::vector<Bvh4Node> leaf_nodes(n);
    for (uint64_t i = 0; i < n; ++i) {
        if (objects[i] >= sv.n_objects) return fail(RTX_ERR_INVALID_ARGUMENT, "rtx_debug_path_bounds: an object index outside Scene.objects");
        uint32_t e = entry_of[objects[i]];
        size_t row = n_rows;
        if (e != kNoEntry) {
            row = (e & kTriEntry) ? prims.size() + (e & ~kTriEntry) : e;
            if (lens[row] == 0u) e = kNoEntry;
        }
        if (e == kNoEntry) row = n_rows;
        entries[i] = e; rows[i] = (uint32_t)row;
        Bvh4Node &w = leaf_nodes[i];
        for (int c = 0; c < 4; ++c) {
            w.a[c] = make_float4(INFINITY, INFINITY, INFINITY, u32_as_f32(0u));
            w.b[c] = make_float4(-INFINITY, -INFINITY, -INFINITY, u32_as_f32(0xFFFFFFFFu));
        }
        if (e != kNoEntry) {
            w.a[0] = make_float4(-INFINITY, -INFINITY, -INFINITY, u32_as_f32(e & ~kTriEntry));
            w.b[0] = make_float4(INFINITY, INFINITY, INFINITY, u32_as_f32((e & kTriEntry) ? (kBvhTriLeaf | 1u) : 1u));
        }
    }
    if (records) {
        std::vector<float4> cr(prims.size()), l32(prims.size()), t32(2 * tri_fidx.size()), geo(2 * tri_fidx.size());
        std::vector<float> s32(prims.empty() ? 0u : (((size_t)sv.n_spheres + 3) & ~(size_t)3) * 4);
        RTX_HIP_CHECK(down(cr.data(), sv.bvh_leaf_cr, cr.size() * sizeof(float4)));
        if (filter_records) {
            RTX_HIP_CHECK(down(l32.data(), sv.bvh_leaf_f32, l32.size() * sizeof(float4)));
            RTX_HIP_CHECK(down(s32.data(), sv.sphere_f32, s32.size() * sizeof(float)));
        }
        RTX_HIP_CHECK(down(t32.data(), sv.tri_f32, t32.size() * sizeof(float4)));
        RTX_HIP_CHECK(down(geo.data(), sv.tri_geo, geo.size() * sizeof(float4)));
        std::memset(records, 0, n * 16 * sizeof(uint32_t));
        for (uint64_t i = 0; i < n; ++i) {
            const uint32_t e = entries[i];
            if (e == kNoEntry) continue;
            if (e & kTriEntry) {
                const size_t r = e & ~kTriEntry;
                const float4 four[4] = { t32[2 * r], t32[2 * r + 1], geo[2 * r], geo[2 * r + 1] };
                std::memcpy(records + 16 * i, four, sizeof four);
            } else {
                std::memcpy(records + 16 * i, &cr[e], sizeof(float4));
                if (!filter_records) continue;
                std::memcpy(records + 16 * i + 4, &l32[e], sizeof(float4));
                const uint32_t k = prims[e];
                if ((size_t)(k | 1u) * 4 + 3 < s32.size()) {
                    const float *f = s32.data() + (size_t)(k & ~1u) * 4 + (k & 1u);
                    const float four[4] = { f[0], f[2], f[4], f[6] };
                    std::memcpy(records + 16 * i + 8, four, sizeof four);
                }
            }
        }
    }
    if (path_data && path_steps) {
        std::vector<BvhQ3Node> q3((form & 2u) && (sv.bvh_flags & 16u) && sv.bvh_q3nodes ? nodes.size() : 0u);
        std::vector<BvhQNode> qn((form & 2u) && q3.empty() ? nodes.size() : 0u);
        RTX_HIP_CHECK(down(q3.data(), sv.bvh_q3nodes, q3.size() * sizeof(BvhQ3Node)));
        RTX_HIP_CHECK(down(qn.data(), sv.bvh_qnodes, qn.size() * sizeof(BvhQNode)));
        std::memset(path_data, 0, n * (size_t)path_steps * 16 * sizeof(uint32_t));
        for (uint64_t i = 0; i < n; ++i) {
            const size_t row = rows[i];
            for (uint32_t k = 0; k < lens[row] && k < path_steps; ++k) {
                const uint32_t link = steps[2 * (row * stride + k)], c = steps[2 * (row * stride + k) + 1], idx = link & ~kBvhFlatNode;
                uint32_t *w = path_data + 16 * ((size_t)i * path_steps + k);
                auto putf = [&](int at, float f) { std::memcpy(w + at, &f, 4); };
                if (!q3.empty()) {
                    const BvhQ3Node &q = q3[idx];
                    w[0] = 2u;
                    putf(1, q.ox); putf(2, q.oy); putf(3, q.oz); putf(4, q.sx); putf(5, q.sy); putf(6, q.sz);
                    w[7] = (q.lox >> (8 * c)) & 255u; w[8] = (q.loy >> (8 * c)) & 255u; w[9] = (q.loz >> (8 * c)) & 255u;
                    w[10] = (q.hix >> (8 * c)) & 255u; w[11] = (q.hiy >> (8 * c)) & 255u; w[12] = (q.hiz >> (8 * c)) & 255u;
                } else if (!qn.empty()) {
                    const BvhQNode &q = qn[idx];
                    w[0] = 3u;
                    putf(1, q.ox); putf(2, q.oy); putf(3, q.sx); putf(4, q.sy); w[5] = q.qx[c]; w[6] = q.qy[c];
                } else if (link & kBvhFlatNode) {
                    w[0] = 1u;
                    putf(1, nodes[idx].a[c].x); putf(2, nodes[idx].a[c].y); putf(3, nodes[idx].a[c].z); putf(4, nodes[idx].a[c].w);
                } else {
                    w[0] = 0u;
                    putf(1, nodes[idx].a[c].x); putf(2, nodes[idx].a[c].y); putf(3, nodes[idx].a[c].z);
                    putf(4, nodes[idx].b[c].x); putf(5, nodes[idx].b[c].y); putf(6, nodes[idx].b[c].z);
                }
                w[15] = link;
            }
        }
    }
    DebugBufs d;
    void *d_sv, *d_rays, *d_entries, *d_rows, *d_lens, *d_steps, *d_best, *d_leaf, *d_out;
    RTX_HIP_CHECK(d.up(&sv, sizeof(SceneView), &d_sv));
    RTX_HIP_CHECK(d.up(rays, n * sizeof(RtxRay), &d_rays));
    RTX_HIP_CHECK(d.up(entries.data(), n * sizeof(uint32_t), &d_entries));
    RTX_HIP_CHECK(d.up(rows.data(), n * sizeof(uint32_t), &d_rows));
    RTX_HIP_CHECK(d.up(lens.data(), lens.size() * sizeof(uint32_t), &d_lens));
    steps.resize(steps.size() + 2, 0u);
    RTX_HIP_CHECK(d.up(steps.data(), steps.size() * sizeof(uint32_t), &d_steps));
    RTX_HIP_CHECK(d.up(best_up, n * sizeof(float), &d_best));
    RTX_HIP_CHECK(d.up(leaf_nodes.data(), n * sizeof(Bvh4Node), &d_leaf));
    RTX_HIP_CHECK(d.up(out, n * 8 * sizeof(uint32_t), &d_out));
    static_assert(sizeof(RtxRay) == sizeof(QueryRay), "RtxRay layout");
    PathBoundsArgs a;
    a.rays = static_cast<const QueryRay *>(d_rays); a.entries = static_cast<const uint32_t *>(d_entries);
    a.rows = static_cast<const uint32_t *>(d_rows); a.lens = static_cast<const uint32_t *>(d_lens);
    a.steps = static_cast<const uint32_t *>(d_steps); a.best_up = static_cast<const float *>(d_best);
    a.leaf_nodes = static_cast<const float4 *>(d_leaf); a.out = static_cast<uint32_t *>(d_out);
    a.n = n; a.stride = stride; a.form = form;
    RTX_HIP_CHECK(launch_debug_path_bounds(static_cast<const SceneView *>(d_sv), a, nullptr));
    RTX_HIP_CHECK(hipMemcpy(out, d_out, n * 8 * sizeof(uint32_t), hipMemcpyDeviceToHost));
    return RTX_OK;
#endif
}

int32_t rtx_debug_tile_lists(RtxSceneHandle h, uint32_t *info, uint32_t *counts, uint32_t *entries, uint64_t max_tiles)
{
#ifndef RTX_LAB
    (void)h; (void)info; (void)counts; (void)entries; (void)max_tiles;
    return fail(RTX_ERR_UNSUPPORTED, "rtx_debug_tile_lists: a lab-library hook (librtx_hip_lab.so)");
#else
    if (!h || !info) return fail(RTX_ERR_INVALID_ARGUMENT, "rtx_debug_tile_lists: null argument");
    const SceneView &sv = h->sv;
    const uint32_t form = h->tl_form, n_tiles = form ? h->tl_tiles : 0u;
    const size_t head = ((size_t)n_tiles * sizeof(uint32_t) + 255) & ~(size_t)255;
    const size_t entry_bytes = form == 1u ? sizeof(TileEntry) : sizeof(uint2);
    const size_t bytes = form == 1u ? bvh_spheres_tile_list_bytes((uint64_t)n_tiles << 6) : wavefront_tile_list_bytes((uint64_t)n_tiles << 6);
    const uint32_t cap = form == 0u ? 0u : (uint32_t)((form == 1u ? bvh_spheres_tile_list_bytes(64) - 256 : wavefront_tile_list_bytes(64) - 256) / entry_bytes);
    const uint32_t words = (uint32_t)(entry_bytes / sizeof(uint32_t));
    const uint32_t head_info[8] = { form, h->tl_tiles_x, n_tiles, cap, words, 0u, 0u, 0u };
    std::memcpy(info, head_info, sizeof head_info);
    if (form == 0u || n_tiles == 0u || (!counts && !entries)) return RTX_OK;
    if (!counts || !entries || max_tiles < n_tiles) return fail(RTX_ERR_INVALID_ARGUMENT, "rtx_debug_tile_lists: counts and entries hold info[2] tiles");
    if ((uint64_t)n_tiles * cap > (1ull << 22)) return fail(RTX_ERR_INVALID_ARGUMENT, "rtx_debug_tile_lists: too large");
    if (!h->tile_lists || h->tile_lists_bytes < bytes || bytes != head + (size_t)n_tiles * cap * entry_bytes)
        return fail(RTX_ERR_HIP, "internal: the handle's tile lists are smaller than the last launch's");
    RTX_HIP_CHECK(hipSetDevice(h->device));
    RTX_HIP_CHECK(hipDeviceSynchronize());
    std::vector<uint32_t> raw(bytes / sizeof(uint32_t));
    RTX_HIP_CHECK(hipMemcpy(raw.data(), h->tile_lists, bytes, hipMemcpyDeviceToHost));
    const bool s_tree = (sv.bvh_flags & 1u) != 0u, t_tree = (sv.bvh_flags & 2u) != 0u;
    std::vector<uint32_t> prims(s_tree ? sv.n_spheres : 0u), sphere_id(sv.n_spheres), tri_fidx(t_tree ? sv.n_tri_tree : 0u);
    std::vector<TriX> tris(t_tree ? sv.n_tris : 0u);
    auto down = [](void *dst, const void *src, size_t b) { return b ? hipMemcpy(dst, src, b, hipMemcpyDeviceToHost) : hipSuccess; };
    RTX_HIP_CHECK(down(prims.data(), sv.bvh_prims, prims.size() * sizeof(uint32_t)));
    RTX_HIP_CHECK(down(sphere_id.data(), sv.sphere_id, sphere_id.size() * sizeof(uint32_t)));
    RTX_HIP_CHECK(down(tri_fidx.data(), sv.tri_fidx, tri_fidx.size() * sizeof(uint32_t)));
    RTX_HIP_CHECK(down(tris.data(), sv.tris, tris.size() * sizeof(TriX)));
    constexpr uint32_t kNoObject = 0xFFFFFFFFu, kSphereEntry = 0x80000000u;
    auto sphere_object = [&](uint32_t prim) { return prim < sphere_id.size() && sphere_id[prim] < sv.n_objects ? sphere_id[prim] : kNoObject; };
    std::memcpy(counts, raw.data(), (size_t)n_tiles * sizeof(uint32_t));
    std::memset(entries, 0, (size_t)n_tiles * cap * 12 * sizeof(uint32_t));
    const uint32_t *lists = raw.data() + head / sizeof(uint32_t);
    for (uint32_t t = 0; t < n_tiles; ++t) {
        if (counts[t] > cap) continue;
        for (uint32_t k = 0; k < counts[t]; ++k) {
            const uint32_t *src = lists + ((size_t)t * cap + k) * words;
            uint32_t *dst = entries + ((size_t)t * cap + k) * 12;
            std::memcpy(dst, src, entry_bytes);
            uint32_t object = kNoObject, kind = 0u;
            if (form == 1u) {
                dst[8] = src[5];
                object = sphere_object(src[4]);
            } else {
                dst[8] = src[1];
                const uint32_t e = src[0] & ~kSphereEntry;
                if (src[0] & kSphereEntry) object = e < prims.size() ? sphere_object(prims[e]) : kNoObject;
                else {
                    kind = 1u;
                    if (e < tri_fidx.size() && tri_fidx[e] < tris.size() && tris[tri_fidx[e]].id < sv.n_objects) object = tris[tri_fidx[e]].id;
                }
            }
            dst[9] = object; dst[10] = kind;
        }
    }
    return RTX_OK;
#endif
}

int32_t rtx_debug_sweep_filter(RtxSceneHandle h, const RtxRay *rays, const uint32_t *objects, uint64_t n, uint32_t *out, double *scene_info)
{
#ifndef RTX_LAB
    (void)h; (void)rays; (void)objects; (void)n; (void)out; (void)scene_info;
    return fail(RTX_ERR_UNSUPPORTED, "rtx_debug_sweep_filter: a lab-library hook (librtx_hip_lab.so)");
#else
    if (!h) return fail(RTX_ERR_INVALID_ARGUMENT, "rtx_debug_sweep_filter: null scene");
    const SceneView &sv = h->sv;
    if (scene_info) {
        uint32_t q = 0, overflow = 0;
        mixed_queue_sizes(&q, &overflow);
        const double info[16] = { sv.sphere_center[0], sv.sphere_center[1], sv.sphere_center[2], sv.sphere_cmax, sv.tri_extent,
                                  (double)sv.n_spheres, (double)sv.n_tri_filter, (double)q, (double)overflow, (double)sv.n_planes,
                                  (double)sv.n_tris, (double)sv.n_objects, (double)sv.n_tri_tree, 0.0, 0.0, 0.0 };
        std::memcpy(scene_info, info, sizeof info);
    }
    if (n == 0) return RTX_OK;
    if (!rays || !out) return fail(RTX_ERR_INVALID_ARGUMENT, "rtx_debug_sweep_filter: null argument");
    if (n > (1ull << 22)) return fail(RTX_ERR_INVALID_ARGUMENT, "rtx_debug_sweep_filter: too large");
    RTX_HIP_CHECK(hipSetDevice(h->device));
    RTX_HIP_CHECK(hipDeviceSynchronize());
    constexpr uint32_t kTriEntry = 0x80000000u, kNoEntry = 0xFFFFFFFFu;
    std::vector<uint32_t> entries;
    if (objects) {
        std::vector<uint32_t> sphere_id(sv.n_spheres), tri_fidx(sv.n_tri_filter);
        std::vector<TriX> tris(sv.n_tri_filter ? sv.n_tris : 0u);
        auto down = [](void *dst, const void *src, size_t bytes) { return bytes ? hipMemcpy(dst, src, bytes, hipMemcpyDeviceToHost) : hipSuccess; };
        RTX_HIP_CHECK(down(sphere_id.data(), sv.sphere_id, sphere_id.size() * sizeof(uint32_t)));
        RTX_HIP_CHECK(down(tri_fidx.data(), sv.tri_fidx, tri_fidx.size() * sizeof(uint32_t)));
        RTX_HIP_CHECK(down(tris.data(), sv.tris, tris.size() * sizeof(TriX)));
        std::vector<uint32_t> entry_of(sv.n_objects, kNoEntry);
        for (size_t k = 0; k < sphere_id.size(); ++k) if (sphere_id[k] < sv.n_objects) entry_of[sphere_id[k]] = (uint32_t)k;
        for (size_t r = 0; r < tri_fidx.size(); ++r)
            if (tri_fidx[r] < tris.size() && tris[tri_fidx[r]].id < sv.n_objects) entry_of[tris[tri_fidx[r]].id] = (uint32_t)r | kTriEntry;
        entries.resize(n);
        for (uint64_t i = 0; i < n; ++i) {
            if (objects[i] >= sv.n_objects) return fail(RTX_ERR_INVALID_ARGUMENT, "rtx_debug_sweep_filter: an object index outside Scene.objects");
            entries[i] = entry_of[objects[i]];
        }
    }
    const size_t out_bytes = n * (objects ? 24 : 4) * sizeof(uint32_t);
    DebugBufs d;
    void *d_sv, *d_rays, *d_entries, *d_out;
    RTX_HIP_CHECK(d.up(&sv, sizeof(SceneView), &d_sv));
    RTX_HIP_CHECK(d.up(rays, n * sizeof(RtxRay), &d_rays));
    RTX_HIP_CHECK(d.up(entries.data(), entries.size() * sizeof(uint32_t), &d_entries));
    RTX_HIP_CHECK(d.up(out, out_bytes, &d_out));
    static_assert(sizeof(RtxRay) == sizeof(QueryRay), "RtxRay layout");
    SweepFilterArgs a;
    a.rays = static_cast<const QueryRay *>(d_rays); a.entries = static_cast<const uint32_t *>(d_entries);
    a.out = static_cast<uint32_t *>(d_out); a.n = n;
    RTX_HIP_CHECK(launch_debug_sweep_filter(static_cast<const SceneView *>(d_sv), a, nullptr));
    RTX_HIP_CHECK(hipMemcpy(out, d_out, out_bytes, hipMemcpyDeviceToHost));
    return RTX_OK;
#endif
}

}
```

### rust-raytracing_amd/csrc/rtx_api_update.hip

```cpp
#include "rtx_host.h"

#include <cstring>

namespace {

template <class T>
hipError_t put_table(T **dst, const std::vector<T> &v)
{
    if (v.empty()) return hipSuccess;
    const hipError_t e = hipMalloc((void **)dst, v.size() * sizeof(T));
    return e != hipSuccess ? e : hipMemcpy(*dst, v.data(), v.size() * sizeof(T), hipMemcpyHostToDevice);
}

int32_t ensure_update_tables(RtxSceneHandle_ *h)
{
    auto &b = h->upd;
    if (!b.d_status) RTX_HIP_CHECK(hipMalloc((void **)&b.d_status, 3 * sizeof(unsigned long long)));
    if (!b.h_status) RTX_HIP_CHECK(hipHostMalloc((void **)&b.h_status, 3 * sizeof(unsigned long long), hipHostMallocDefault));
    if (b.valid) return RTX_OK;
    drop_update_tables(h);
    const RefitTables &t = h->refit;
    std::vector<float> box32;
    std::vector<double> reach;
    derive_all_spheres(h->objects.data(), h->objects.size(), t, h->sv.n_spheres, box32, reach, h->hidden.empty() ? nullptr : h->hidden.data());
    RTX_HIP_CHECK(put_table(&b.box32, box32));
    RTX_HIP_CHECK(put_table(&b.reach, reach));
    RTX_HIP_CHECK(put_table(&b.levels, t.level_nodes));
    b.valid = true;
    return RTX_OK;
}

int32_t ensure_mesh_tables(RtxSceneHandle_ *h)
{
    auto &b = h->upd;
    if (b.mesh_valid) return RTX_OK;
    const RefitTables &t = h->refit;
    std::vector<float> tribox32;
    std::vector<double> tri_reach;
    derive_all_triangles(h->objects.data(), h->objects.size(), t, tribox32, tri_reach, h->hidden.empty() ? nullptr : h->hidden.data());
    RTX_HIP_CHECK(put_table(&b.tribox32, tribox32));
    RTX_HIP_CHECK(put_table(&b.tri_reach, tri_reach));
    if (!b.all_levels) RTX_HIP_CHECK(put_table(&b.all_levels, t.all_level_nodes));
    b.mesh_valid = true;
    return RTX_OK;
}

int32_t apply_plan(RtxSceneHandle_ *h, UpdatePlan &plan, hipStream_t stream)
{
    auto &b = h->upd;
    if (int32_t rc = ensure_update_tables(h)) return rc;
    if (plan.tri_geom) if (int32_t rc = ensure_mesh_tables(h)) return rc;
    const RefitTables &t = h->refit;
    plan.capture = plan.visibility && !b.keep_valid;
    if (plan.capture) {
        if (!t.all_level_nodes.empty() && !b.all_levels) RTX_HIP_CHECK(put_table(&b.all_levels, t.all_level_nodes));
        if (h->sv.n_bvh_nodes) RTX_HIP_CHECK(hipMalloc((void **)&b.keep, (size_t)h->sv.n_bvh_nodes * kKeepWords * sizeof(uint32_t)));
        b.keep_valid = true;
    }
    const size_t ne = plan.entries.size(), bytes = ne * sizeof(UpdateEntry);
    if (b.h_cap < ne) {
        if (b.h_entries) { RTX_HIP_CHECK(hipHostFree(b.h_entries)); b.h_entries = nullptr; b.h_cap = 0; }
        RTX_HIP_CHECK(hipHostMalloc((void **)&b.h_entries, bytes, hipHostMallocDefault));
        b.h_cap = ne;
    }
    if (b.d_cap < ne) {
        if (b.d_entries) { RTX_HIP_CHECK(hipFree(b.d_entries)); b.d_entries = nullptr; b.d_cap = 0; }
        RTX_HIP_CHECK(hipMalloc((void **)&b.d_entries, bytes));
        b.d_cap = ne;
    }
    std::memcpy(b.h_entries, plan.entries.data(), bytes);
    {
        if (int32_t rc = adopt_stream(h, stream)) return rc;
        DoneGuard done{h, stream};
        const SceneView &sv = h->sv;
        RTX_HIP_CHECK(hipMemcpyAsync(b.d_entries, b.h_entries, bytes, hipMemcpyHostToDevice, stream));
        const size_t status_bytes = (plan.any_tri ? 3 : 2) * sizeof(unsigned long long);
        RTX_HIP_CHECK(hipMemsetAsync(b.d_status, 0, status_bytes, stream));
        UpdateArgs u = update_args(sv, t, b.d_entries, b.box32, b.reach, b.tribox32, b.tri_reach, plan.tri_geom, b.keep);
        u.status = b.d_status;
        hipError_t scene_update_launch = hipSuccess;
        run_update(u, t, plan, b.levels, b.all_levels, sv.n_spheres, sv.n_tris,
                   [&](const UpdateArgs &a) { return (scene_update_launch = launch_scene_update(a, stream)) == hipSuccess; });
        RTX_HIP_CHECK(scene_update_launch);
        RTX_HIP_CHECK(hipMemcpyAsync(b.h_status, b.d_status, status_bytes, hipMemcpyDeviceToHost, stream));
        RTX_HIP_CHECK(hipStreamSynchronize(stream));
    }
    if (b.h_status[0] & (kUpdateStatusNoQ3 | kUpdateStatusNoQ)) { plan.how = RTX_UPDATED_REBUILT; return RTX_OK; }
    if (plan.any_sphere) { std::memcpy(&h->sv.sphere_cmax, &b.h_status[1], sizeof(double)); h->sv_dirty = true; }
    if (plan.any_tri) { std::memcpy(&h->sv.tri_extent, &b.h_status[2], sizeof(double)); h->sv_dirty = true; }
    return RTX_OK;
}

int32_t repack_objects(RtxSceneHandle_ *h, std::vector<RtxObject> &all, std::vector<uint8_t> &hidden, hipStream_t stream)
{
    RtxScene sc{};
    sc.config = h->cfg;
    sc.camera = h->cam;
    sc.n_objects = all.size();
    sc.objects = all.data();
    PackedScene p;
    if (int32_t rc = pack_scene(&sc, p)) return rc;
    if (int32_t rc = upload_packed(h, p)) return rc;
    h->objects.swap(all);
    h->hidden.clear();
    std::vector<uint64_t> idx;
    for (size_t k = 0; k < hidden.size(); ++k) if (hidden[k]) idx.push_back(k);
    if (idx.empty()) return RTX_OK;
    const std::vector<uint8_t> none(h->objects.size(), 0);
    UpdatePlan plan;
    if (int32_t rc = plan_visibility(h->objects, none, h->refit, 0.0, idx.data(), idx.size(), 0u, plan)) return rc;
    if (!(h->sv.sphere_cmax < 1.0e14)) plan.any_sphere = false;
    if (int32_t rc = apply_plan(h, plan, stream)) return rc;
    h->hidden.swap(hidden);
    h->hidden.resize(h->objects.size(), 0);
    if (plan.how == RTX_UPDATED_REBUILT) return fail(RTX_ERR_UNSUPPORTED, "hidden objects: a 64-byte node of the fresh pack has no encoding without them");
    return RTX_OK;
}

std::vector<uint8_t> hidden_bytes(const RtxSceneHandle_ *h, size_t n)
{
    std::vector<uint8_t> v = h->hidden;
    v.resize(n, 0);
    return v;
}

}

extern "C" {

int32_t rtx_scene_append_objects(RtxSceneHandle scene, const RtxObject *objects, uint64_t n_objects)
{
    if (!scene || (n_objects && !objects)) return fail(RTX_ERR_INVALID_ARGUMENT, "rtx_scene_append_objects: null argument");
    if (n_objects == 0) return RTX_OK;
    if (scene->objects.size() + n_objects > 0xFFFFFFF0ull) return fail(RTX_ERR_INVALID_ARGUMENT, "rtx_scene_append_objects: too many objects");
    RTX_HIP_CHECK(hipSetDevice(scene->device));
    RTX_HIP_CHECK(hipDeviceSynchronize());
    if (int32_t rc = check_watchdog(scene, true)) return rc;
    std::vector<RtxObject> all = scene->objects;
    all.insert(all.end(), objects, objects + n_objects);
    std::vector<uint8_t> hidden = hidden_bytes(scene, all.size());
    return repack_objects(scene, all, hidden, nullptr);
}

int32_t rtx_scene_update_objects(RtxSceneHandle h, const uint64_t *indices, const RtxObject *objects, uint64_t n, uint32_t mode,
                                 void *stream_, uint32_t *how)
{
    if (how) *how = RTX_UPDATED_NOTHING;
    if (!h) return fail(RTX_ERR_INVALID_ARGUMENT, "rtx_scene_update_objects: null scene");
    UpdatePlan plan;
    if (int32_t rc = plan_update(h->objects, h->refit, h->sv.sphere_cmax, indices, objects, n, mode, plan, h->hidden.empty() ? nullptr : h->hidden.data()))
        return rc;
    if (plan.entries.empty()) return RTX_OK;
    RTX_HIP_CHECK(hipSetDevice(h->device));
    if (int32_t rc = check_watchdog(h, true)) return rc;
    hipStream_t stream = static_cast<hipStream_t>(stream_);
    if (plan.how != RTX_UPDATED_REBUILT) {
        if (int32_t rc = apply_plan(h, plan, stream)) return rc;
        if (plan.how != RTX_UPDATED_REBUILT)
            for (const UpdateEntry &e : plan.entries) std::memcpy(&h->objects[e.object], &e.kind, sizeof(RtxObject));
    }
    if (plan.how == RTX_UPDATED_REBUILT) {
        RTX_HIP_CHECK(hipDeviceSynchronize());
        std::vector<RtxObject> all = h->objects;
        for (const UpdateEntry &e : plan.entries) std::memcpy(&all[e.object], &e.kind, sizeof(RtxObject));
        std::vector<uint8_t> hidden = hidden_bytes(h, all.size());
        if (int32_t rc = repack_objects(h, all, hidden, stream)) return rc;
    }
    if (how) *how = plan.how;
    return RTX_OK;
}

int32_t rtx_scene_set_visible(RtxSceneHandle h, const uint64_t *indices, uint64_t n, uint32_t visible, void *stream_, uint32_t *how)
{
    if (how) *how = RTX_UPDATED_NOTHING;
    if (!h) return fail(RTX_ERR_INVALID_ARGUMENT, "rtx_scene_set_visible: null scene");
    std::vector<uint8_t> hidden = hidden_bytes(h, h->objects.size());
    UpdatePlan plan;
    if (int32_t rc = plan_visibility(h->objects, hidden, h->refit, h->sv.sphere_cmax, indices, n, visible, plan)) return rc;
    if (plan.entries.empty()) return RTX_OK;
    RTX_HIP_CHECK(hipSetDevice(h->device));
    if (int32_t rc = check_watchdog(h, true)) return rc;
    hipStream_t stream = static_cast<hipStream_t>(stream_);
    if (h->hidden.empty()) h->hidden.assign(h->objects.size(), 0);
    if (plan.how != RTX_UPDATED_REBUILT) if (int32_t rc = apply_plan(h, plan, stream)) return rc;
    for (const UpdateEntry &e : plan.entries) hidden[e.object] = (e.tri & kEntryHide) ? 1 : 0;
    if (plan.how == RTX_UPDATED_REBUILT) {
        RTX_HIP_CHECK(hipDeviceSynchronize());
        std::vector<RtxObject> all = h->objects;
        if (int32_t rc = repack_objects(h, all, hidden, stream)) return rc;
    } else h->hidden.swap(hidden);
    if (how) *how = plan.how;
    return RTX_OK;
}

int32_t rtx_scene_get_visible(RtxSceneHandle h, uint8_t *mask)
{
    if (!h || (!mask && !h->objects.empty())) return fail(RTX_ERR_INVALID_ARGUMENT, "rtx_scene_get_visible: null argument");
    for (size_t k = 0; k < h->objects.size(); ++k) mask[k] = (k < h->hidden.size() && h->hidden[k]) ? 0 : 1;
    return RTX_OK;
}

}
```

### rust-raytracing_amd/csrc/rtx_bvh_spheres.hip

```cpp
#include "rtx_launch.h"
#include "rtx_spk_units.h"
#include "rtx_traverse.h"

#include <cmath>

namespace rtx {

#ifndef RTX_SPH_WAVES
#define RTX_SPH_WAVES 4
#endif
constexpr int kSphWavesPerSimd = RTX_SPH_WAVES;
constexpr int kSphStack = 30;

struct SphSurvivor {
    double px, py, pz, dx, dy, dz;
    uint32_t ridx;
    uint32_t first_id;
    uint64_t key;
};
static_assert(sizeof(SphSurvivor) == 64, "SphSurvivor must be one 64-byte line");
struct SphQueue {
    SphSurvivor *rec;
    const uint32_t *perm;
    unsigned long long *count;
    unsigned long long capacity;
    uint32_t cut_walkers;
};
constexpr uint32_t kSphQueueChunk = 512;
#ifndef RTX_SPH_CUT
#define RTX_SPH_CUT 24
#endif
#ifndef RTX_SPH_CUT_DONE
#define RTX_SPH_CUT_DONE 32
#endif
#ifndef RTX_SPH_LEAF_LANES
#define RTX_SPH_LEAF_LANES 8
#endif
#ifndef RTX_ROUND_GLOBAL
#define RTX_ROUND_GLOBAL 1
#endif
#ifndef RTX_ROUND_CARRY_KEY
#define RTX_ROUND_CARRY_KEY 1
#endif
#ifndef RTX_ROUND_DRAW
#define RTX_ROUND_DRAW 1
#endif
constexpr bool kRoundGlobal = RTX_ROUND_GLOBAL != 0;
constexpr uint32_t kSphLeafLanes = RTX_SPH_LEAF_LANES;
constexpr uint32_t kSphCutWalkers = RTX_SPH_CUT;
constexpr uint32_t kSphCutDone = RTX_SPH_CUT_DONE;

__device__ __forceinline__ void sph_queue_append(const SphQueue &sq, Counters *__restrict__ ctr, bool go, const RayState &r,
                                                 uint32_t ridx, uint32_t first_id, uint32_t lane,
                                                 unsigned long long &out_next, unsigned long long &out_end)
{
    const unsigned long long m = __ballot(go);
    const uint32_t n = (uint32_t)__popcll(m);
    if (n == 0u) return;
    const unsigned long long rem = out_end - out_next;
    unsigned long long base2 = 0;
    if (rem < (unsigned long long)n) {
        if (lane == 0) base2 = atomicAdd(sq.count, (unsigned long long)kSphQueueChunk);
        base2 = ((unsigned long long)__builtin_amdgcn_readfirstlane((uint32_t)(base2 >> 32)) << 32) |
                __builtin_amdgcn_readfirstlane((uint32_t)base2);
    }
    if (go) {
        const unsigned long long k = bvh_mbcnt(m);
        const unsigned long long slot = k < rem ? out_next + k : base2 + (k - rem);
        if (slot < sq.capacity) {
            double4 *p = reinterpret_cast<double4 *>(sq.rec + slot);
            p[0] = make_double4(r.pos.x, r.pos.y, r.pos.z, r.dir.x);
            uint2 tail;
            tail.x = ridx; tail.y = first_id;
#if RTX_ROUND_CARRY_KEY
            p[1] = make_double4(r.dir.y, r.dir.z, __longlong_as_double(((long long)tail.y << 32) | (long long)tail.x),
                                __longlong_as_double((long long)r.key));
#else
            p[1] = make_double4(r.dir.y, r.dir.z, __longlong_as_double(((long long)tail.y << 32) | (long long)tail.x), 0.0);
#endif
        } else {
            atomicAdd(&ctr[1].pad_, 1ull);
        }
    }
    if (rem < (unsigned long long)n) { out_next = base2 + ((unsigned long long)n - rem); out_end = base2 + kSphQueueChunk; }
    else out_next += n;
}

__device__ __forceinline__ void sph_queue_close(const SphQueue &sq, uint32_t lane, unsigned long long out_next, unsigned long long out_end)
{
    for (unsigned long long s = out_next + lane; s < out_end; s += 64ull)
        if (s < sq.capacity) sq.rec[s].ridx = kNone;
}

template <bool SPILL, int MODE, int Q3 = 0>
__global__ __launch_bounds__(kBvhThreads, kSphWavesPerSimd) void trace_bvh_spheres_kernel(const SceneView *__restrict__ svp,
                                                                             const RowsView *__restrict__ rvp,
                                                                             double *__restrict__ samples, Counters *__restrict__ ctr,
                                                                             unsigned long long *__restrict__ work_counter,
                                                                             const float4 *__restrict__ nodes, const LeafArrays la,
                                                                             uint32_t *__restrict__ spill, uint32_t spill_entries,
                                                                             const SphQueue sq)
{
    constexpr int STACK = kSphStack;
    const SceneView &sv = *svp;
    const RowsView &rv = *rvp;
    __shared__ uint32_t lds_stack[STACK + 1][kBvhThreads];
    __shared__ uint32_t lds_q[2 * kSphQueue][kBvhThreads];
    uint32_t *const lq = &lds_q[0][0];
    const uint32_t tid = threadIdx.x;
    const uint32_t lane = tid & 63u;
    const size_t spill_stride = (size_t)gridDim.x * kBvhThreads, glane = (size_t)blockIdx.x * kBvhThreads + tid;
    const uint32_t bounce_limit = sv.max_bounces >= 0xFFFFFFF0ull ? 0xFFFFFFF0u : (uint32_t)sv.max_bounces + 1u;

    const unsigned long long n_rays = MODE == 2 ? (*sq.count < sq.capacity ? *sq.count : sq.capacity) : rv.n_rays;
    unsigned long long wave_next = 0, wave_end = 0;
    unsigned long long out_next = 0, out_end = 0;
    bool queue_empty = false;
    bool alive = false;
    RayState r;
    uint32_t ridx = 0;
    uint32_t first_id = 0;
    unsigned long long segs = 0, box_tests = 0, leaf_filters = 0, exact = 0;
    float best_up = __builtin_inff();
    uint32_t qcnt = 0, nbox = 0, nleaf = 0, w_node = kNone, w_sp = 0;
    bool overflow = false, walked = false, midwalk = false;
#if defined(RTX_LAB) && defined(RTX_SPH_PROFILE)
    unsigned long long rtx_prof = 0, t_prev = 0;
#define RTX_PROF_PASS , rtx_prof
#else
#define RTX_PROF_PASS
#endif
    const uint32_t cut_walkers = MODE == 1 ? 0u : sq.cut_walkers;

    for (;;) {
        const unsigned long long idle_mask = __ballot(!alive);
        if (idle_mask != 0ull) {
            if (wave_next >= wave_end && !queue_empty) {
                unsigned long long base = 0;
                if (lane == 0) base = atomicAdd(work_counter, (unsigned long long)rv.grab);
                base = ((unsigned long long)__builtin_amdgcn_readfirstlane((uint32_t)(base >> 32)) << 32) |
                       __builtin_amdgcn_readfirstlane((uint32_t)base);
                wave_next = base;
                wave_end = base + rv.grab < n_rays ? base + rv.grab : n_rays;
                if (base >= n_rays) { queue_empty = true; wave_next = wave_end = 0; }
            }
            if (!alive && wave_next < wave_end) {
                const unsigned long long my = wave_next + bvh_mbcnt(idle_mask);
                bool valid = my < wave_end;
                uint32_t pl = 0, smp = 0;
                if constexpr (MODE == 2) {
                    double4 s0 = make_double4(0., 0., 0., 0.), s1 = s0;
                    if (valid) {
                        const double4 *p = reinterpret_cast<const double4 *>(sq.rec + (sq.perm ? (unsigned long long)sq.perm[my] : my));
// ... 43 lines not shown
#if defined(RTX_LAB) && defined(RTX_SPH_PROFILE) && RTX_SPH_PROFILE >= 10
        const unsigned long long t_w0 = __builtin_amdgcn_s_memtime();
        if (RTX_SPH_PROFILE == 11 && lane == 0 && t_prev != 0ull) rtx_prof += (t_w0 - t_prev) >> 6;
#endif
        const uint32_t n_alive = (uint32_t)__popcll(__ballot(alive));
        if (!midwalk) { best_up = __builtin_inff(); qcnt = 0; nbox = 0; nleaf = 0; overflow = false; walked = false; w_node = kNone; w_sp = 0; }
        RayX rx;
        if (alive) {
            rx = make_rayx(r.pos, r.dir);
            const float omax = fmaxf(fmaxf(__builtin_fabsf((float)r.pos.x), __builtin_fabsf((float)r.pos.y)),
                                     __builtin_fabsf((float)r.pos.z));
            const bool in32 = omax <= sv.bvh_origin_limit;
            const bool in64 = !in32 && omax <= sv.bvh_origin_limit * kBvhRange64;
            if (in32 || in64) {
                SphereRay sr;
                sphere_ray_from(sv, r.pos, r.dir, sr);
                const V3 dirn = rx.dirn;
                if (!midwalk) w_node = sv.bvh_root;
                if constexpr (Q3) {
                    Ray32 q0;
                    make_ray32(r.pos, dirn, (double)sv.bvh_inv_max, q0);
                    Ray32S q;
                    q.ix = q0.ix; q.iy = q0.iy; q.iz = q0.iz; q.nx = q0.nx; q.ny = q0.ny; q.nz = q0.nz;
                    q.e = ray32_slack(q0, in32);
                    if constexpr (Q3 == 2)
                        sphere_walk_phased<STACK, SPILL, RTX_WALK_INNER != 0>(nodes, la.sphere_f32, la.sphere_prims, q, sr, w_node, w_sp, &lds_stack[0][0],
                                                         lq, tid, spill, spill_entries, spill_stride, glane, best_up, qcnt,
                                                         overflow, nbox, nleaf, cut_walkers, kSphCutDone, n_alive, kSphLeafLanes RTX_PROF_PASS);
                    else
                        sphere_walk_resumable<STACK, SPILL, true>(nodes, la.sphere_f32, la.sphere_prims, q, sr, w_node, w_sp, &lds_stack[0][0],
                                                                  lq, tid, spill, spill_entries, spill_stride, glane, best_up, qcnt,
                                                                  overflow, nbox, nleaf, cut_walkers, kSphCutDone, n_alive);
                } else if (in32) {
                    Ray32 q;
                    make_ray32(r.pos, dirn, (double)sv.bvh_inv_max, q);
                    sphere_walk_resumable<STACK, SPILL, false>(nodes, la.sphere_f32, la.sphere_prims, q, sr, w_node, w_sp, &lds_stack[0][0],
                                                               lq, tid, spill, spill_entries, spill_stride, glane, best_up, qcnt,
                                                               overflow, nbox, nleaf, cut_walkers, kSphCutDone, n_alive);
                } else {
                    Ray64 q;
                    make_ray64(r.pos, dirn, (double)sv.bvh_inv_max, q);
                    sphere_walk_resumable<STACK, SPILL, false>(nodes, la.sphere_f32, la.sphere_prims, q, sr, w_node, w_sp, &lds_stack[0][0],
                                                               lq, tid, spill, spill_entries, spill_stride, glane, best_up, qcnt,
                                                               overflow, nbox, nleaf, cut_walkers, kSphCutDone, n_alive);
                }
                walked = true;
                midwalk = w_node != kNone;
            }
        }
#if defined(RTX_LAB) && defined(RTX_SPH_PROFILE) && RTX_SPH_PROFILE >= 10
        {
            const unsigned long long t_w1 = __builtin_amdgcn_s_memtime();
            if (RTX_SPH_PROFILE == 10 && lane == 0) rtx_prof += (t_w1 - t_w0) >> 6;
            t_prev = t_w1;
        }
#endif
#if defined(RTX_LAB) && defined(RTX_SPH_PROFILE)
        {
            const unsigned long long fm = __ballot(alive && !midwalk);
            if (RTX_SPH_PROFILE == 1 && fm != 0ull && (uint32_t)(__ffsll((long long)fm) - 1) == lane) rtx_prof += 1;
            if (RTX_SPH_PROFILE == 2) {
                uint32_t mx = alive && !midwalk && walked && !overflow ? qcnt : 0u;
                for (int off = 32; off > 0; off >>= 1) { const uint32_t o = (uint32_t)__shfl_xor((int)mx, off, 64); mx = mx > o ? mx : o; }
                if (lane == 0) rtx_prof += mx;
            }
            if (RTX_SPH_PROFILE == 8 && alive && !midwalk && walked && !overflow) rtx_prof += qcnt;
        }
#endif
        if (alive && !midwalk) {
            Hit h;
            hit_init(h);
            ++segs;
            box_tests += nbox;
            leaf_filters += nleaf;
            if (walked && !overflow) {
#pragma unroll 1
                for (uint32_t e = 0; e < qcnt; ++e) {
                    if (__uint_as_float(lq[(size_t)(kSphQueue + e) * kBvhThreads + tid]) <= best_up) {
                        const uint32_t idx = lq[(size_t)e * kBvhThreads + tid];
                        double t;
                        if (sphere_distance(la.spheres[idx], rx, &t)) hit_consider(h, t, la.sphere_ids[idx], 0, idx);
                        exact += 1;
                    }
                }
            } else {
                for (uint32_t k = 0; k < sv.n_spheres; ++k) {
                    double t;
                    if (sphere_distance(la.spheres[k], rx, &t)) hit_consider(h, t, la.sphere_ids[k], 0, k);
                }
                exact += sv.n_spheres;
            }
            for (uint32_t k = 0; k < sv.n_planes; ++k) {
                double t;
                if (plane_distance(sv.planes[k], rx, &t)) hit_consider(h, t, sv.planes[k].id, 1, k);
            }
            for (uint32_t k = 0; k < sv.n_tri_filter; ++k) {
                const uint32_t tk = la.tri_fidx[k];
                double t;
                if (triangle_distance(la.tris[tk], rx, &t)) hit_consider(h, t, la.tris[tk].id, 2, tk);
            }
            exact += sv.n_planes + sv.n_tri_filter;

            bool done = true;
            if (h.id != kNone) {
#if RTX_ROUND_DRAW
                r.draw = 6u + 2u * r.bounce;
#endif
                advance_and_shade<kRoundGlobal>(sv, h, r);
                first_id = h.id;
                done = (r.bounce >= bounce_limit) || light_is_zero(r);
            }
            if (done) {
                store_sample<kRoundGlobal>(samples, rv, ridx, r.result);
                alive = false;
            }
        }
        if constexpr (MODE == 1) {
            sph_queue_append(sq, ctr, alive, r, ridx, first_id, lane, out_next, out_end);
            alive = false;
        }
    }
    if constexpr (MODE == 1) sph_queue_close(sq, lane, out_next, out_end);
#if defined(RTX_LAB) && defined(RTX_SPH_PROFILE)
    if (MODE == 2) exact = rtx_prof;
#endif
    unsigned long long filt = box_tests + leaf_filters;
#pragma unroll
    for (int off = 32; off > 0; off >>= 1) {
        segs += __shfl_xor(segs, off, 64);
        exact += __shfl_xor(exact, off, 64);
        filt += __shfl_xor(filt, off, 64);
        box_tests += __shfl_xor(box_tests, off, 64);
    }
    if (lane == 0) {
        const uint32_t shard = (blockIdx.x * (kBvhThreads >> 6) + (tid >> 6)) & (kCounterShards - 1);
        if (segs) atomicAdd(&ctr[shard].segments, segs);
        if (exact) atomicAdd(&ctr[shard].exact_tests, exact);
        if (filt) atomicAdd(&ctr[shard].filter_tests, filt);
        if (box_tests) atomicAdd(&ctr[2 + (shard % (kCounterShards - 2))].pad_, box_tests);
    }
}

constexpr int kSpkStack = 63;
#ifndef RTX_SPK_WAVES
#define RTX_SPK_WAVES 4
#endif
constexpr int kSpkWaves = RTX_SPK_WAVES;
#ifndef RTX_SPK_LAZY_RAY
#define RTX_SPK_LAZY_RAY 1
#endif
#ifndef RTX_SPK_UNITS
#define RTX_SPK_UNITS 1
#endif
#ifdef RTX_LAB
constexpr uint32_t kSphNoPackets = 1u;
#endif



template <int SGN>
__device__ __forceinline__ void sph_packet_walk(const PkConst4 cnodes, const PkConst4 csph, const PkConstU32 cprims, uint32_t root,
                                                const Ray32S &q, const SphereRay &sr, uint32_t *lq, uint32_t tid, uint32_t lane,
                                                float &best_up, uint32_t &qcnt, bool &overflow, uint32_t &nbox, uint32_t &nleaf)
{
    int stk = 0;
    uint32_t sp = 0, node = __builtin_amdgcn_readfirstlane(root);
    while (node != kNone) {
        const PkConst4 np = cnodes + 8 * (size_t)node;
        float4 a[4], b[4];
#pragma unroll
        for (int c = 0; c < 4; ++c) { a[c] = np[c]; b[c] = np[4 + c]; }
        uint32_t lnk[4], cnt[4];
        float tc[4];
        unsigned long long hm[4];
#pragma unroll
        for (int c = 0; c < 4; ++c) {
            lnk[c] = pk_bits(a[c].w);
            cnt[c] = pk_bits(b[c].w);
            float tn, tf;
            if (SGN < 8) {
                const float nx_ = (SGN & 1) ? b[c].x : a[c].x, fx_ = (SGN & 1) ? a[c].x : b[c].x;
                const float ny_ = (SGN & 2) ? b[c].y : a[c].y, fy_ = (SGN & 2) ? a[c].y : b[c].y;
                const float nz_ = (SGN & 4) ? b[c].z : a[c].z, fz_ = (SGN & 4) ? a[c].z : b[c].z;
                tn = fmaxf(fmaxf(__builtin_fmaf(nx_, q.ix, q.nx), __builtin_fmaf(ny_, q.iy, q.ny)), fmaxf(__builtin_fmaf(nz_, q.iz, q.nz), 0.0f));
                tf = fminf(fminf(__builtin_fmaf(fx_, q.ix, q.nx), __builtin_fmaf(fy_, q.iy, q.ny)), __builtin_fmaf(fz_, q.iz, q.nz));
            } else {
                const float x0 = __builtin_fmaf(a[c].x, q.ix, q.nx), x1 = __builtin_fmaf(b[c].x, q.ix, q.nx);
                const float y0 = __builtin_fmaf(a[c].y, q.iy, q.ny), y1 = __builtin_fmaf(b[c].y, q.iy, q.ny);
                const float z0 = __builtin_fmaf(a[c].z, q.iz, q.nz), z1 = __builtin_fmaf(b[c].z, q.iz, q.nz);
                tn = fmaxf(fmaxf(fminf(x0, x1), fminf(y0, y1)), fmaxf(fminf(z0, z1), 0.0f));
                tf = fminf(fminf(fmaxf(x0, x1), fmaxf(y0, y1)), fmaxf(z0, z1));
            }
            tc[c] = __builtin_fmaf(tn, 1.0f - 4.76837158e-7f, -q.e);
            const float tf_hi = __builtin_fmaf(tf, 1.0f + 4.76837158e-7f, q.e);
            hm[c] = __builtin_amdgcn_ballot_w64(tc[c] <= fminf(tf_hi, best_up));
        }
        if (best_up >= 0.0f) nbox += 4;
        if (((cnt[0] | cnt[1] | cnt[2] | cnt[3]) & 0xFFFFu) != 0u) {
            uint32_t leafmask = 0;
#pragma unroll
            for (int c = 0; c < 4; ++c)
                if (cnt[c] - 1u < 0xFFFFu && hm[c] != 0ull) leafmask |= 1u << c;
            while (leafmask != 0u) {
                const uint32_t c = (uint32_t)__builtin_ctz(leafmask);
                leafmask &= leafmask - 1u;
                const uint32_t first = c == 0 ? lnk[0] : (c == 1 ? lnk[1] : (c == 2 ? lnk[2] : lnk[3]));
                const uint32_t n = (c == 0 ? cnt[0] : (c == 1 ? cnt[1] : (c == 2 ? cnt[2] : cnt[3]))) & 0xFFFFu;
                const unsigned long long m = c == 0 ? hm[0] : (c == 1 ? hm[1] : (c == 2 ? hm[2] : hm[3]));
                const bool in = ((m >> lane) & 1ull) != 0ull;
                if (in) nleaf += n;
                for (uint32_t j = 0; j < n; ++j) {
                    const float4 rec = csph[first + j];
                    const uint32_t prim = cprims[first + j];
                    if (!in) continue;
                    sph_packet_leaf_test(rec, prim, sr, lq, tid, best_up, qcnt, overflow);
                }
            }
#pragma unroll
            for (int c = 0; c < 4; ++c) hm[c] &= __builtin_amdgcn_ballot_w64(tc[c] <= best_up);
        }
#ifndef RTX_SPK_FAST1
#define RTX_SPK_FAST1 2
#endif
#if RTX_SPK_FAST1
        {
            uint32_t ib = 0;
#pragma unroll
            for (int c = 0; c < 4; ++c) ib |= (cnt[c] == 0u && hm[c] != 0ull) ? 1u << c : 0u;
            if ((ib & (ib - 1u)) == 0u) {
                node = ib == 0u ? kNone : (ib == 1u ? lnk[0] : (ib == 2u ? lnk[1] : (ib == 4u ? lnk[2] : lnk[3])));
                if (node == kNone && sp != 0u) {
                    sp -= 1;
                    node = (uint32_t)__builtin_amdgcn_readlane(stk, (int)sp);
                }
                continue;
            }
#if RTX_SPK_FAST1 >= 2
            if (__builtin_popcount(ib) == 2) {
                uint32_t far_link = 0;
#define RTX_SPK_PAIR(A, B)                                                                                                        \
                {                                                                                                                   \
                    const int ka = (int)__builtin_amdgcn_readlane(__float_as_uint(tc[A]), (int)__builtin_ctzll(hm[A]));            \
                    const int kb = (int)__builtin_amdgcn_readlane(__float_as_uint(tc[B]), (int)__builtin_ctzll(hm[B]));            \
                    const bool sw = kb < ka;                                                                                        \
                    node = sw ? lnk[B] : lnk[A];                                                                                    \
                    far_link = sw ? lnk[A] : lnk[B];                                                                                \
                }
                switch (ib) {
                    case 3u: RTX_SPK_PAIR(0, 1) break;
                    case 5u: RTX_SPK_PAIR(0, 2) break;
                    case 9u: RTX_SPK_PAIR(0, 3) break;
                    case 6u: RTX_SPK_PAIR(1, 2) break;
                    case 10u: RTX_SPK_PAIR(1, 3) break;
                    default: RTX_SPK_PAIR(2, 3) break;
                }
#undef RTX_SPK_PAIR
                stk = rtx_writelane((int)far_link, (int)sp, stk);
                sp += 1u;
                continue;
            }
#endif
        }
#endif
        int key[4];
        uint32_t kl[4];
        constexpr int kFar = 0x7F800000;
#pragma unroll
        for (int c = 0; c < 4; ++c) {
            const unsigned long long m = cnt[c] == 0u ? hm[c] : 0ull;
            const int k = (int)__builtin_amdgcn_readlane(__float_as_uint(tc[c]), (int)__builtin_ctzll(m | 0x8000000000000000ull));
            key[c] = m != 0ull ? k : kFar;
            kl[c] = lnk[c];
        }
#define RTX_CSWAP(i, j) { if (key[j] < key[i]) { int tk = key[i]; key[i] = key[j]; key[j] = tk; uint32_t tl = kl[i]; kl[i] = kl[j]; kl[j] = tl; } }
        RTX_CSWAP(0, 1) RTX_CSWAP(2, 3) RTX_CSWAP(0, 2) RTX_CSWAP(1, 3) RTX_CSWAP(1, 2)
#undef RTX_CSWAP
        stk = rtx_writelane((int)kl[3], (int)sp, stk); sp += key[3] < kFar ? 1u : 0u;
        stk = rtx_writelane((int)kl[2], (int)sp, stk); sp += key[2] < kFar ? 1u : 0u;
        stk = rtx_writelane((int)kl[1], (int)sp, stk); sp += key[1] < kFar ? 1u : 0u;
        node = key[0] < kFar ? kl[0] : kNone;
        if (node == kNone && sp != 0u) {
            sp -= 1;
            node = (uint32_t)__builtin_amdgcn_readlane(stk, (int)sp);
        }
    }
}


__global__ __launch_bounds__(kBvhThreads, kSpkWaves) void trace_sph_packet_kernel(const SceneView *__restrict__ svp,
                                                                                  const RowsView *__restrict__ rvp,
                                                                                  double *__restrict__ samples, Counters *__restrict__ ctr,
                                                                                  unsigned long long *__restrict__ work_counter,
                                                                                  const float4 *__restrict__ nodes, const LeafArrays la,
                                                                                  const SphQueue sq, const TileLists tl)
{
    const SceneView &sv = *svp;
    const RowsView &rv = *rvp;
    __shared__ uint32_t lds_q[2 * kSphQueue][kBvhThreads];
    uint32_t *const lq = &lds_q[0][0];
    const uint32_t tid = threadIdx.x, lane = tid & 63u;
    const uint32_t bounce_limit = sv.max_bounces >= 0xFFFFFFF0ull ? 0xFFFFFFF0u : (uint32_t)sv.max_bounces + 1u;
    const unsigned long long n_rays = rv.n_rays;
    const PkConst4 cnodes = pk_const(nodes), csph = pk_const(la.sphere_f32);
    const PkConstU32 cprims = pk_const(la.sphere_prims);
#if !RTX_SPK_UNITS
    unsigned long long wave_next = 0, wave_end = 0;
#endif
    unsigned long long out_next = 0, out_end = 0;
    unsigned long long segs = 0, box_tests = 0, leaf_filters = 0, exact = 0;

#ifndef RTX_SPK_GRAB_MUL
#define RTX_SPK_GRAB_MUL 2
#endif
    const unsigned long long pk_grab = (unsigned long long)rv.grab * RTX_SPK_GRAB_MUL;
#if RTX_SPK_UNITS
    const uint32_t per_sample = rv.div_per_sample.d, n_tiles = per_sample >> 6;
    const uint32_t unit_run = (uint32_t)(pk_grab >> 6) != 0u ? (uint32_t)(pk_grab >> 6) : 1u;
    const unsigned long long n_units = n_rays != 0ull ? spk_unit_count(n_tiles, rv.n_samples, unit_run) : 0ull;
#endif
    for (;;) {
#if RTX_SPK_UNITS
        unsigned long long unit = 0;
        if (lane == 0) unit = atomicAdd(work_counter, 1ull);
        unit = ((unsigned long long)__builtin_amdgcn_readfirstlane((uint32_t)(unit >> 32)) << 32) |
               __builtin_amdgcn_readfirstlane((uint32_t)unit);
        if (unit >= n_units) break;
        const SpkUnit wu = spk_unit((uint32_t)unit, n_tiles, rv.n_samples, unit_run);
        const uint32_t tile_of = wu.tile;
        uint32_t list_n = kTileListWalk;
        if (tl.count != nullptr) list_n = pk_const(tl.count)[tile_of];
        const uint32_t tile_ray = tile_of * 64u + lane;
        uint32_t pl = 0, smp0 = 0;
        const bool valid = ray_index_to_pixel_tiled(rv, tile_ray, pl, smp0);
        uint64_t pixel_half = 0;
        V3 focal_point = mk(0., 0., 0.);
        if (valid) {
            const uint32_t k = fastdiv(pl, rv.div_width), x = pl - k * rv.width;
            pixel_half = rng_key_pixel(sv.seed, (uint64_t)image_row(rv, k) * rv.width + x);
            focal_point = primary_focal_point(sv, rv, pl);
        }
        const PkConst4 ent = pk_const(reinterpret_cast<const float4 *>(tl.entries + (size_t)tile_of * kTileListCap));
#pragma unroll 1
        for (uint32_t us = 0; us < wu.count; ++us) {
            const uint32_t smp = wu.first + us;
            const uint32_t ridx = smp * per_sample + tile_ray;
            bool alive = valid;
            RayState r;
            if (alive) gen_primary_at(sv, pixel_half, focal_point, rv.sample_begin + smp, r);
            else { r.pos = mk(0., 0., 0.); r.dir = mk(1., 0., 0.); r.result = mk(0., 0., 0.); r.light = mk(1., 1., 1.); r.key = 0; r.draw = 6; r.bounce = 0; }
#else
        {
            unsigned long long base = 0;
            if (lane == 0) base = atomicAdd(work_counter, pk_grab);
            base = ((unsigned long long)__builtin_amdgcn_readfirstlane((uint32_t)(base >> 32)) << 32) |
                   __builtin_amdgcn_readfirstlane((uint32_t)base);
            if (base >= n_rays) break;
            wave_next = base;
            wave_end = base + pk_grab < n_rays ? base + pk_grab : n_rays;
        }
        for (; wave_next < wave_end; wave_next += 64ull) {
            const unsigned long long my = wave_next + lane;
            uint32_t pl = 0, smp = 0;
            bool alive = ray_index_to_pixel_tiled(rv, my, pl, smp);
            uint32_t list_n = kTileListWalk;
            const uint32_t tile_of = __builtin_amdgcn_readfirstlane((uint32_t)(((uint32_t)my - smp * rv.div_per_sample.d) >> 6));
            if (tl.count != nullptr) list_n = pk_const(tl.count)[tile_of];
            const PkConst4 ent = pk_const(reinterpret_cast<const float4 *>(tl.entries + (size_t)tile_of * kTileListCap));
            RayState r;
            if (alive) gen_primary(sv, rv, pl, rv.sample_begin + smp, r);
            else { r.pos = mk(0., 0., 0.); r.dir = mk(1., 0., 0.); r.result = mk(0., 0., 0.); r.light = mk(1., 1., 1.); r.key = 0; r.draw = 6; r.bounce = 0; }
            const uint32_t ridx = (uint32_t)my;
#endif
            const RayX rx = make_rayx(r.pos, r.dir);

            float best_up = -__builtin_inff();
            uint32_t qcnt = 0, nbox = 0, nleaf = 0;
            bool overflow = false, walked = false, in32 = false;
            SphereRay sr;
            sr.px = sr.py = sr.pz = sr.dx = sr.dy = sr.dz = sr.Kg = sr.K = 0.f; sr.c0 = __builtin_inff();
#if !RTX_SPK_LAZY_RAY
            Ray32S q;
            q.ix = q.iy = q.iz = 1.0f; q.nx = q.ny = q.nz = 0.0f; q.e = 0.0f;
#endif
            if (alive) {
                const float omax = fmaxf(fmaxf(__builtin_fabsf((float)r.pos.x), __builtin_fabsf((float)r.pos.y)),
                                         __builtin_fabsf((float)r.pos.z));
                in32 = omax <= sv.bvh_origin_limit;
                if (in32 || omax <= sv.bvh_origin_limit * kBvhRange64) {
                    sphere_ray_from(sv, r.pos, r.dir, sr);
#if !RTX_SPK_LAZY_RAY
                    Ray32 q0;
                    make_ray32(r.pos, rx.dirn, (double)sv.bvh_inv_max, q0);
                    q.ix = q0.ix; q.iy = q0.iy; q.iz = q0.iz; q.nx = q0.nx; q.ny = q0.ny; q.nz = q0.nz;
                    q.e = ray32_slack(q0, in32);
#endif
                    best_up = __builtin_inff();
                    walked = true;
                }
            }
            const unsigned long long wm = __ballot(walked);
            if (wm != 0ull && list_n != kTileListWalk) {
                for (uint32_t k = 0; k < list_n; ++k) {
                    const float4 rec = ent[2 * k], tail = ent[2 * k + 1];
                    const float t_lb = tail.y;
                    const bool in = walked && t_lb <= best_up;
                    if (__ballot(in) == 0ull) break;
                    if (in) {
                        nleaf += 1;
                        sph_packet_leaf_test(rec, __float_as_uint(tail.x), sr, lq, tid, best_up, qcnt, overflow);
                    }
                }
            } else if (wm != 0ull) {
#if RTX_SPK_LAZY_RAY
                Ray32S q;
                q.ix = q.iy = q.iz = 1.0f; q.nx = q.ny = q.nz = 0.0f; q.e = 0.0f;
                if (walked) {
                    Ray32 q0;
                    make_ray32(r.pos, rx.dirn, (double)sv.bvh_inv_max, q0);
                    q.ix = q0.ix; q.iy = q0.iy; q.iz = q0.iz; q.nx = q0.nx; q.ny = q0.ny; q.nz = q0.nz;
                    q.e = ray32_slack(q0, in32);
                }
#endif
                const uint32_t my_sgn = (q.ix < 0.0f ? 1u : 0u) | (q.iy < 0.0f ? 2u : 0u) | (q.iz < 0.0f ? 4u : 0u);
                const uint32_t sgn = __builtin_amdgcn_readlane(my_sgn, (int)(__ffsll((long long)wm) - 1));
                const uint32_t oct = __ballot(walked && my_sgn != sgn) == 0ull ? sgn : 8u;
#define RTX_SPK_WALK(S) sph_packet_walk<S>(cnodes, csph, cprims, sv.bvh_root, q, sr, lq, tid, lane, best_up, qcnt, overflow, nbox, nleaf)
                switch (oct) {
                    case 0: RTX_SPK_WALK(0); break;
                    case 1: RTX_SPK_WALK(1); break;
                    case 2: RTX_SPK_WALK(2); break;
                    case 3: RTX_SPK_WALK(3); break;
                    case 4: RTX_SPK_WALK(4); break;
                    case 5: RTX_SPK_WALK(5); break;
                    case 6: RTX_SPK_WALK(6); break;
                    case 7: RTX_SPK_WALK(7); break;
                    default: RTX_SPK_WALK(8); break;
                }
#undef RTX_SPK_WALK
            }
            uint32_t first_id = 0;
            if (alive) {
                Hit h;
                hit_init(h);
                ++segs;
                box_tests += nbox;
                leaf_filters += nleaf;
                if (walked && !overflow) {
#pragma unroll 1
                    for (uint32_t e = 0; e < qcnt; ++e) {
                        if (__uint_as_float(lq[(size_t)(kSphQueue + e) * kBvhThreads + tid]) <= best_up) {
                            const uint32_t idx = lq[(size_t)e * kBvhThreads + tid];
                            double t;
                            if (sphere_distance(la.spheres[idx], rx, &t)) hit_consider(h, t, la.sphere_ids[idx], 0, idx);
                            exact += 1;
                        }
                    }
                } else {
                    for (uint32_t k = 0; k < sv.n_spheres; ++k) {
                        double t;
                        if (sphere_distance(la.spheres[k], rx, &t)) hit_consider(h, t, la.sphere_ids[k], 0, k);
                    }
                    exact += sv.n_spheres;
                }
                for (uint32_t k = 0; k < sv.n_planes; ++k) {
                    double t;
                    if (plane_distance(sv.planes[k], rx, &t)) hit_consider(h, t, sv.planes[k].id, 1, k);
                }
                for (uint32_t k = 0; k < sv.n_tri_filter; ++k) {
                    const uint32_t tk = la.tri_fidx[k];
                    double t;
                    if (triangle_distance(la.tris[tk], rx, &t)) hit_consider(h, t, la.tris[tk].id, 2, tk);
                }
                exact += sv.n_planes + sv.n_tri_filter;

                bool done = true;
                if (h.id != kNone) {
                    advance_and_shade<kRoundGlobal>(sv, h, r);
                    first_id = h.id;
                    done = (r.bounce >= bounce_limit) || light_is_zero(r);
                }
                if (done) {
                    store_sample<kRoundGlobal>(samples, rv, ridx, r.result);
                    alive = false;
                }
            }
            sph_queue_append(sq, ctr, alive, r, ridx, first_id, lane, out_next, out_end);
        }
    }
    sph_queue_close(sq, lane, out_next, out_end);
    unsigned long long filt = box_tests + leaf_filters;
#pragma unroll
    for (int off = 32; off > 0; off >>= 1) {
        segs += __shfl_xor(segs, off, 64);
        exact += __shfl_xor(exact, off, 64);
        filt += __shfl_xor(filt, off, 64);
        box_tests += __shfl_xor(box_tests, off, 64);
    }
    if (lane == 0) {
        const uint32_t shard = (blockIdx.x * (kBvhThreads >> 6) + (tid >> 6)) & (kCounterShards - 1);
        if (segs) atomicAdd(&ctr[shard].segments, segs);
        if (exact) atomicAdd(&ctr[shard].exact_tests, exact);
        if (filt) atomicAdd(&ctr[shard].filter_tests, filt);
        if (box_tests) atomicAdd(&ctr[2 + (shard % (kCounterShards - 2))].pad_, box_tests);
    }
}

uint32_t bvh_spheres_spill_entries(const SceneView &sv)
{
    const uint32_t need = 3u * sv.bvh_depth + 2u;
    return need > (uint32_t)kSphStack ? need - (uint32_t)kSphStack : 0u;
}

size_t bvh_spheres_spill_bytes(const SceneView &sv, int n_cus)
{
    return (size_t)bvh_spheres_spill_entries(sv) * (size_t)n_cus * kSphWavesPerSimd * kBvhThreads * sizeof(uint32_t);
}

static uint64_t sph_queue_capacity(uint64_t n_rays, int n_cus)
{
    const int wpc = kSphWavesPerSimd > kSpkWaves ? kSphWavesPerSimd : kSpkWaves;
    return n_rays + (uint64_t)n_cus * wpc * (kBvhThreads / 64) * kSphQueueChunk + kSphQueueChunk;
}

size_t bvh_spheres_tile_list_bytes(uint64_t rays_per_sample)
{
    const uint64_t n_tiles = rays_per_sample >> 6;
    return (size_t)(((n_tiles * sizeof(uint32_t) + 255) & ~(uint64_t)255) + n_tiles * kTileListCap * sizeof(TileEntry));
}

size_t bvh_spheres_queue_bytes(uint64_t n_rays, int n_cus)
{
    const uint64_t cap = sph_queue_capacity(n_rays, n_cus);
    return (size_t)(cap * sizeof(SphSurvivor) + 2 * 256);
}

static bool sph_packets_ok(const SceneView &sv, bool tiled)
{
    return tiled && 3u * sv.bvh_depth + 2u <= (uint32_t)kSpkStack;
}

bool bvh_spheres_two_stage_ok(const SceneView &sv, bool tiled)
{
#ifdef RTX_LAB
    (void)sv; (void)tiled;
    return true;
#else
    return sph_packets_ok(sv, tiled);
#endif
}

hipError_t launch_trace_bvh_spheres(const SceneView *d_sv, const SceneView &sv, const RowsView *d_rv, const RowsView &rv,
                                    double *samples, Counters *counters, unsigned long long *work_counter, uint32_t *spill, int n_cus,
                                    void *queue_mem, uint32_t flags, hipStream_t stream, Counters *stage1_snapshot, hipEvent_t stage1_done,
                                    void *tile_list_mem, bool build_tile_lists)
{
    const uint64_t want = (rv.n_rays + kBvhThreads - 1) / kBvhThreads;
    const uint64_t cap = (uint64_t)n_cus * kSphWavesPerSimd;
    const uint32_t blocks = (uint32_t)(want < cap ? want : cap);
    if (blocks == 0) return hipSuccess;
    LeafArrays la;
    la.sphere_f32 = sv.bvh_leaf_cr; la.sphere_prims = sv.bvh_prims; la.spheres = sv.spheres; la.sphere_ids = sv.sphere_id;
    la.tri_f32 = sv.tri_f32; la.tri_fidx = sv.tri_fidx; la.tris = sv.tris;
    const uint32_t spill_entries = spill ? bvh_spheres_spill_entries(sv) : 0u;
    const bool deep = spill_entries != 0u;
    const float4 *nodes = reinterpret_cast<const float4 *>(sv.bvh_nodes);
    SphQueue sq{};
    sq.cut_walkers = (sv.tuning & RTX_TUNE_NO_CUT) != 0u ? 0u : kSphCutWalkers;
    const float4 *q3nodes = reinterpret_cast<const float4 *>(sv.bvh_q3nodes);
#ifdef RTX_LAB
    const bool q3 = (sv.bvh_flags & 16u) != 0u && sv.bvh_q3nodes != nullptr && (sv.tuning & RTX_TUNE_NO_QNODES) == 0u;
    const bool inl = (sv.tuning & RTX_TUNE_INLINE_LEAVES) != 0u;
#else
    if ((sv.bvh_flags & 16u) == 0u || sv.bvh_q3nodes == nullptr) return hipErrorInvalidValue;
    (void)flags;
#endif
    const bool tiled = rv.tiles_x != 0u && (rv.n_rays & 63ull) == 0ull;
    if (!queue_mem || sv.max_bounces == 0) {
#ifdef RTX_LAB
        auto kernel = !q3 ? (deep ? trace_bvh_spheres_kernel<true, 0> : trace_bvh_spheres_kernel<false, 0>)
                          : inl ? (deep ? trace_bvh_spheres_kernel<true, 0, 1> : trace_bvh_spheres_kernel<false, 0, 1>)
                                : (deep ? trace_bvh_spheres_kernel<true, 0, 2> : trace_bvh_spheres_kernel<false, 0, 2>);
        hipLaunchKernelGGL(kernel, dim3(blocks), dim3(kBvhThreads), 0, stream, d_sv, d_rv, samples, counters, work_counter,
                           q3 ? q3nodes : nodes, la, spill, spill_entries, sq);
#else
        auto kernel = deep ? trace_bvh_spheres_kernel<true, 0, 2> : trace_bvh_spheres_kernel<false, 0, 2>;
        hipLaunchKernelGGL(kernel, dim3(blocks), dim3(kBvhThreads), 0, stream, d_sv, d_rv, samples, counters, work_counter,
                           q3nodes, la, spill, spill_entries, sq);
#endif
        return hipGetLastError();
    }
    const uint64_t capacity = sph_queue_capacity(rv.n_rays, n_cus);
    char *p = static_cast<char *>(queue_mem);
    unsigned long long *ctrs = reinterpret_cast<unsigned long long *>(p);
    sq.rec = reinterpret_cast<SphSurvivor *>(p + 256);
    sq.count = ctrs;
    sq.capacity = capacity;
    hipError_t e = hipMemsetAsync(ctrs, 0, 2 * sizeof(unsigned long long), stream);
    if (e != hipSuccess) return e;
#ifdef RTX_LAB
    if ((flags & kSphNoPackets) != 0u || !sph_packets_ok(sv, tiled)) {
        auto k1 = deep ? trace_bvh_spheres_kernel<true, 1> : trace_bvh_spheres_kernel<false, 1>;
        hipLaunchKernelGGL(k1, dim3(blocks), dim3(kBvhThreads), 0, stream, d_sv, d_rv, samples, counters, work_counter, nodes, la, spill,
                           spill_entries, sq);
    } else
#else
    if (!sph_packets_ok(sv, tiled)) return hipErrorInvalidValue;
#endif
    {
        const uint64_t pcap = (uint64_t)n_cus * kSpkWaves;
        const uint32_t pblocks = (uint32_t)(want < pcap ? want : pcap);
        TileLists tl{};
        if (tile_list_mem && tiled && (sv.tuning & RTX_TUNE_NO_TILE_LISTS) == 0u) {
            const uint32_t n_tiles = (uint32_t)((rv.n_rays / rv.n_samples) >> 6);
            tl.count = reinterpret_cast<uint32_t *>(tile_list_mem);
            tl.entries = reinterpret_cast<TileEntry *>(static_cast<char *>(tile_list_mem) + (((size_t)n_tiles * sizeof(uint32_t) + 255) & ~(size_t)255));
            if (build_tile_lists && (e = launch_build_sphere_tile_lists(d_sv, d_rv, sv, n_tiles, tl.count, tl.entries, stream)) != hipSuccess) return e;
        }
        hipLaunchKernelGGL(trace_sph_packet_kernel, dim3(pblocks), dim3(kBvhThreads), 0, stream, d_sv, d_rv, samples, counters, work_counter,
                           nodes, la, sq, tl);
    }
    if ((e = hipGetLastError()) != hipSuccess) return e;
    if (stage1_snapshot && (e = hipMemcpyAsync(stage1_snapshot, counters, sizeof(Counters) * kCounterShards, hipMemcpyDeviceToDevice, stream)) != hipSuccess) return e;
    if (stage1_done && (e = hipEventRecord(stage1_done, stream)) != hipSuccess) return e;
#ifdef RTX_LAB
    if (!q3 || inl) {
        auto k2 = !q3 ? (deep ? trace_bvh_spheres_kernel<true, 2> : trace_bvh_spheres_kernel<false, 2>)
                      : (deep ? trace_bvh_spheres_kernel<true, 2, 1> : trace_bvh_spheres_kernel<false, 2, 1>);
        hipLaunchKernelGGL(k2, dim3(blocks), dim3(kBvhThreads), 0, stream, d_sv, d_rv, samples, counters, ctrs + 1, q3 ? q3nodes : nodes, la, spill,
                           spill_entries, sq);
        return hipGetLastError();
    }
#endif
    auto k2 = deep ? trace_bvh_spheres_kernel<true, 2, 2> : trace_bvh_spheres_kernel<false, 2, 2>;
    hipLaunchKernelGGL(k2, dim3(blocks), dim3(kBvhThreads), 0, stream, d_sv, d_rv, samples, counters, ctrs + 1, q3nodes, la, spill, spill_entries, sq);
    return hipGetLastError();
}

}
```

### rust-raytracing_amd/csrc/rtx_host.h

```cpp
#pragma once

#include "rtx_launch.h"
#include "rtx_pack.h"

using namespace rtx;
using namespace rtx::host;

#define RTX_HIP_CHECK(expr)                                                                              \
    do {                                                                                                 \
        hipError_t e_ = (expr);                                                                          \
        if (e_ != hipSuccess)                                                                            \
            return fail(e_ == hipErrorOutOfMemory ? RTX_ERR_OUT_OF_MEMORY : RTX_ERR_HIP,                 \
                        std::string(#expr) + ": " + hipGetErrorString(e_));                              \
    } while (0)

struct RtxSceneHandle_ {
    int device = 0;
    int n_cus = 0;
    RtxConfig cfg{};
    RtxCamera cam{};
    SceneView sv{};
    std::vector<RtxObject> objects;
    std::vector<uint8_t> hidden;
    std::vector<void *> scene_allocs;
    RefitTables refit;
    struct UpdateBufs {
        bool valid = false;
        uint32_t *levels = nullptr; float *box32 = nullptr; double *reach = nullptr;
        bool mesh_valid = false;
        uint32_t *all_levels = nullptr; float *tribox32 = nullptr; double *tri_reach = nullptr;
        bool keep_valid = false;
        uint32_t *keep = nullptr;
        UpdateEntry *h_entries = nullptr; size_t h_cap = 0;
        UpdateEntry *d_entries = nullptr; size_t d_cap = 0;
        unsigned long long *d_status = nullptr, *h_status = nullptr;
    } upd;
    double *samples = nullptr;  size_t samples_bytes = 0;
    double *acc = nullptr;      size_t acc_bytes = 0;
    double *tables = nullptr;   size_t tables_doubles = 0;
    double *h_tables = nullptr; size_t h_tables_doubles = 0;
    double *state = nullptr;    size_t state_bytes = 0;
    void *wf_state = nullptr;   size_t wf_bytes = 0;
    void *tile_lists = nullptr; size_t tile_lists_bytes = 0;
#ifdef RTX_LAB
    uint32_t tl_form = 0, tl_tiles_x = 0, tl_tiles = 0;
#endif
    PathStep *transcript = nullptr; uint32_t *transcript_counts = nullptr; uint32_t transcript_steps = 0;
    Counters *counters = nullptr;
    unsigned long long *work_counter = nullptr;
    SceneView *d_sv = nullptr;  bool sv_dirty = true;
    RowsView *d_rv = nullptr;
    hipEvent_t ev[4] = { nullptr, nullptr, nullptr, nullptr };
    struct SecondHalf {
        hipStream_t stream = nullptr;
        hipEvent_t fork = nullptr, join = nullptr, stage1_done = nullptr;
        Counters *counters = nullptr, *counters_stage1 = nullptr;
        unsigned long long *work_counter = nullptr;
        RowsView *d_rv = nullptr;
        double *state = nullptr;    size_t state_bytes = 0;
        void *queue = nullptr;      size_t queue_bytes = 0;
    } half2;
    Counters *counters_stage1 = nullptr;
    size_t scratch_limit = 0;
    hipStream_t last_stream = nullptr;
    bool have_last_stream = false;
    hipEvent_t ev_done = nullptr;
    bool have_done = false;
    unsigned long long *h_watchdog = nullptr;
    hipEvent_t ev_watchdog = nullptr;
    bool watchdog_pending = false;
    uint32_t t_w = 0, t_h = 0, t_rb = 0, t_rs = 0, t_blk = 0, t_nr = 0;
    double t_fov = 0.0;
    bool t_valid = false;
};

RTX_HOST_BEGIN

inline size_t nonzero_mask_bytes(uint64_t n_rays) { return (size_t)((n_rays + 31) / 32) * sizeof(uint32_t); }

struct SampleRange { uint64_t begin = 0, n = 0; double *sum = nullptr, *sum_sq = nullptr; };

struct DoneGuard {
    RtxSceneHandle_ *h; hipStream_t stream;
    ~DoneGuard() {
        if (hipEventRecord(h->ev_done, stream) == hipSuccess) h->have_done = true;
        else { (void)hipGetLastError(); (void)hipDeviceSynchronize(); h->have_done = false; }
    }
};

int usable_device_count();
void drop_update_tables(RtxSceneHandle_ *h);
int32_t upload_packed(RtxSceneHandle_ *h, const PackedScene &p);
int32_t check_watchdog(RtxSceneHandle_ *h, bool wait);
int32_t adopt_stream(RtxSceneHandle_ *h, hipStream_t stream);
int32_t render_band(RtxSceneHandle_ *h, uint32_t width, uint32_t height, uint32_t row_begin, uint32_t row_stride, uint32_t row_block,
                    uint32_t n_rows, double *d_out_rgb, void *stream_, RtxStats *stats, const SampleRange *accumulate = nullptr);

RTX_HOST_END
```

Measured before the change: 4252 Mrays/s.

## Pool sphere hits in LDS for full-wave shading and reuse tile lists across renders

Adds a per-wave LDS pool to the two-stage sphere BVH kernel. Lanes with hits are parked in the pool until there are 64, and then the whole wave shades them together. The goal is to cut divergence in the shading and queue-append step. Separately, tile lists are cached under a key of scene generation, camera and band parameters, so repeated renders of an unchanged scene skip the list-build pass. The risks are extra LDS use, which can lower occupancy, and stale lists if some path that mutates the scene does not call touch_scene.

```diff
diff --git a/rust-raytracing_amd/__init__.py b/rust-raytracing_amd/__init__.py
--- a/rust-raytracing_amd/__init__.py
+++ b/rust-raytracing_amd/__init__.py
@@ -514,7 +514,7 @@
             self._check(self._lib.rtx_debug_tile_lists(self._h, info.ctypes.data, count.ctypes.data, ent.ctypes.data, n_tiles))
         obj = ent[:, :, 9].astype(np.int64)
         obj[obj == 0xFFFFFFFF] = -1
-        return {"form": form, "tiles_x": tiles_x, "n_tiles": n_tiles, "cap": cap, "count": count, "raw": ent[:, :, :8].copy(),
+        return {"form": form, "tiles_x": tiles_x, "n_tiles": n_tiles, "cap": cap, "builds": int(info[5]), "count": count, "raw": ent[:, :, :8].copy(),
                 "t_lb": np.ascontiguousarray(ent[:, :, 8]).view(np.float32), "object": obj, "is_record": ent[:, :, 10] == 1}
 
     def debug_sweep_filter(self, origins, directions, objects=None):
diff --git a/rust-raytracing_amd/build.py b/rust-raytracing_amd/build.py
--- a/rust-raytracing_amd/build.py
+++ b/rust-raytracing_amd/build.py
@@ -12,7 +12,7 @@
 SOURCES = ["rtx_kernels.hip", "rtx_bvh_spheres.hip", "rtx_bvh_mesh.hip", "rtx_wavefront.hip", "rtx_query.hip", "rtx_update.hip", "rtx_pack.hip",
            "rtx_api.hip", "rtx_api_update.hip", "rtx_api_debug.hip"]
 HEADERS = ["rtx_math.h", "rtx_scene.h", "rtx_bvh.h", "rtx_device.h", "rtx_traverse.h", "rtx_mesh_step.h", "rtx_wavefront.h",
-           "rtx_launch.h", "rtx_refit.h", "rtx_pack.h", "rtx_host.h", "rtx_spk_units.h"]
+           "rtx_launch.h", "rtx_refit.h", "rtx_pack.h", "rtx_host.h", "rtx_spk_units.h", "rtx_spk_pool.h"]
 FLAGS = ["--offload-arch=gfx950", "-O3", "-std=c++17", "-fPIC", "-ffp-contract=off",
          "-fno-fast-math", "-Wall", "-Wno-unused-function"]
 LAB_FLAGS = ["-DRTX_LAB"]
diff --git a/rust-raytracing_amd/csrc/rtx_api.hip b/rust-raytracing_amd/csrc/rtx_api.hip
--- a/rust-raytracing_amd/csrc/rtx_api.hip
+++ b/rust-raytracing_amd/csrc/rtx_api.hip
@@ -112,6 +112,7 @@
 
 int32_t upload_packed(RtxSceneHandle_ *h, const PackedScene &p)
 {
+    touch_scene(h);
     const SceneView sv_before = h->sv;
     std::vector<void *> old_allocs;
     old_allocs.swap(h->scene_allocs);
@@ -413,6 +414,7 @@
     if (!scene || !config) return fail(RTX_ERR_INVALID_ARGUMENT, "rtx_scene_set_config: null argument");
     if (int32_t rc = check_config(*config)) return rc;
     if (int32_t rc = check_watchdog(scene, false)) return rc;
+    touch_scene(scene);
     apply_config(scene, *config);
     return RTX_OK;
 }
@@ -420,6 +422,7 @@
 int32_t rtx_scene_set_scratch_limit(RtxSceneHandle scene, uint64_t bytes)
 {
     if (!scene) return fail(RTX_ERR_INVALID_ARGUMENT, "rtx_scene_set_scratch_limit: null scene");
+    touch_scene(scene);
     scene->scratch_limit = (size_t)bytes;
     return RTX_OK;
 }
@@ -428,6 +431,7 @@
 {
     if (!scene || !camera) return fail(RTX_ERR_INVALID_ARGUMENT, "rtx_scene_set_camera: null argument");
     if (int32_t rc = check_watchdog(scene, false)) return rc;
+    touch_scene(scene);
     scene->cam = *camera;
     scene->sv.cam_pos = mk(camera->position[0], camera->position[1], camera->position[2]);
     scene->sv.to_world_x = mk(camera->to_world_space[0], camera->to_world_space[1], camera->to_world_space[2]);
@@ -575,6 +579,23 @@
                   ((tuning & RTX_TUNE_HALVES) != 0u || plan.per_sample64 * spp <= kHalvesBelowRays);
 }
 
+#ifndef RTX_TILE_LIST_REUSE
+#define RTX_TILE_LIST_REUSE 1
+#endif
+bool tile_list_key_equal(const RtxSceneHandle_::TileListKey &a, const RtxSceneHandle_::TileListKey &b)
+{
+    return a.valid && b.valid && a.scene_gen == b.scene_gen && std::memcmp(&a.cam, &b.cam, sizeof(RtxCamera)) == 0 &&
+           a.width == b.width && a.height == b.height && a.row_begin == b.row_begin && a.row_stride == b.row_stride &&
+           a.row_block == b.row_block && a.n_rows == b.n_rows && a.tiles_x == b.tiles_x && a.kernel == b.kernel && a.tuning == b.tuning &&
+           a.buffer == b.buffer && a.bytes == b.bytes;
+}
+
+int32_t grow_tile_lists(RtxSceneHandle_ *h, size_t bytes)
+{
+    if (!h->tile_lists || h->tile_lists_bytes < bytes) h->tl_key.valid = false;
+    return grow(&h->tile_lists, &h->tile_lists_bytes, bytes);
+}
+
 int32_t grow_scratch(RtxSceneHandle_ *h, const BandPlan &plan, uint32_t npix, uint64_t spp, bool own_acc)
 {
     const uint32_t kernel = plan.kernel;
@@ -594,13 +615,13 @@
     if (plan.spheres_two_stage) {
         if (int32_t rc = grow(&h->wf_state, &h->wf_bytes, bvh_spheres_queue_bytes(batch_rays, h->n_cus))) return rc;
         if (plan.tile_list_bytes != 0)
-            if (int32_t rc = grow(&h->tile_lists, &h->tile_lists_bytes, (size_t)plan.tile_list_bytes)) return rc;
+            if (int32_t rc = grow_tile_lists(h, (size_t)plan.tile_list_bytes)) return rc;
     }
     if (kernel == RTX_KERNEL_WAVEFRONT) {
         if (int32_t rc = grow((void **)&h->state, &h->state_bytes, wavefront_spill_bytes(h->sv, h->n_cus))) return rc;
         if (int32_t rc = grow(&h->wf_state, &h->wf_bytes, wavefront_state_bytes(batch_rays, wavefront_levels(h->sv)))) return rc;
         if (plan.tile_list_bytes != 0)
-            if (int32_t rc = grow(&h->tile_lists, &h->tile_lists_bytes, (size_t)plan.tile_list_bytes)) return rc;
+            if (int32_t rc = grow_tile_lists(h, (size_t)plan.tile_list_bytes)) return rc;
     }
     return RTX_OK;
 }
@@ -688,10 +709,14 @@
     return RTX_OK;
 }
 
-int32_t launch_batch(RtxSceneHandle_ *h, const BandPlan &plan, const RowsView &rv, bool first_batch, hipStream_t stream, bool stats)
+int32_t launch_batch(RtxSceneHandle_ *h, const BandPlan &plan, const RowsView &rv, bool build_lists, hipStream_t stream, bool stats)
 {
     const uint32_t kernel = plan.kernel, tuning = h->cfg.tuning;
     uint32_t *const state = reinterpret_cast<uint32_t *>(h->state);
+#ifdef RTX_LAB
+    if (build_lists && plan.tile_list_bytes != 0 && (kernel == RTX_KERNEL_WAVEFRONT || (kernel == RTX_KERNEL_BVH && plan.spheres_two_stage)))
+        ++h->tl_builds;
+#endif
     if (kernel != RTX_KERNEL_EXACT && kernel != RTX_KERNEL_WAVEFRONT)
         RTX_HIP_CHECK(hipMemsetAsync(h->work_counter, 0, sizeof(unsigned long long), stream));
     if (kernel == RTX_KERNEL_EXACT) {
@@ -702,7 +727,7 @@
 #endif
     } else if (kernel == RTX_KERNEL_WAVEFRONT) {
         RTX_HIP_CHECK(launch_trace_wavefront(h->d_sv, h->sv, h->d_rv, rv, h->samples, h->wf_state, h->counters, state, h->n_cus, stream,
-                                             plan.tile_list_bytes != 0 ? h->tile_lists : nullptr, first_batch));
+                                             plan.tile_list_bytes != 0 ? h->tile_lists : nullptr, build_lists));
     } else if (kernel == RTX_KERNEL_BVH_REGROUP) {
         RTX_HIP_CHECK(launch_trace_bvh_mesh(h->d_sv, h->sv, h->d_rv, rv, h->samples, h->counters, h->work_counter, state, h->n_cus, stream));
     } else if (kernel == RTX_KERNEL_BVH) {
@@ -710,7 +735,7 @@
         RTX_HIP_CHECK(launch_trace_bvh_spheres(h->d_sv, h->sv, h->d_rv, rv, h->samples, h->counters, h->work_counter, state, h->n_cus,
                                                two ? h->wf_state : nullptr, sphere_flags(tuning), stream,
                                                stats && two ? h->counters_stage1 : nullptr, stats && two ? h->ev[3] : nullptr,
-                                               two && plan.tile_list_bytes != 0 ? h->tile_lists : nullptr, first_batch));
+                                               two && plan.tile_list_bytes != 0 ? h->tile_lists : nullptr, build_lists));
     } else {
         RTX_HIP_CHECK(launch_trace_mixed(h->d_sv, h->sv, h->d_rv, rv, h->samples, h->state, h->counters, h->work_counter, h->n_cus,
                                          kernel == RTX_KERNEL_MIXED_VERIFY, stream));
@@ -719,7 +744,7 @@
 }
 
 int32_t launch_batches(RtxSceneHandle_ *h, const BandPlan &plan, RowsView rv, const SampleRange &sr, double *d_out_rgb, hipStream_t stream,
-                       bool stats, BandRun &run)
+                       bool stats, BandRun &run, bool lists_current)
 {
     const uint64_t spp = sr.n;
     const bool accumulate = sr.sum != nullptr;
@@ -732,7 +757,7 @@
         RTX_HIP_CHECK(hipMemcpyAsync(h->d_rv, &rv, sizeof(RowsView), hipMemcpyHostToDevice, stream));
         RTX_HIP_CHECK(hipMemsetAsync(rv.nonzero, 0, nonzero_mask_bytes(rv.n_rays), stream));
         if (stats) RTX_HIP_CHECK(hipEventRecord(h->ev[0], stream));
-        if (int32_t rc = launch_batch(h, plan, rv, s0 == 0, stream, stats)) return rc;
+        if (int32_t rc = launch_batch(h, plan, rv, s0 == 0 && !lists_current, stream, stats)) return rc;
         ++run.launches;
         if (stats) RTX_HIP_CHECK(hipEventRecord(h->ev[1], stream));
         if (accumulate)
@@ -856,6 +881,16 @@
 #endif
     if (int32_t rc = ensure_tables(h, width, height, row_begin, row_stride, row_block, n_rows, stream)) return rc;
     if (int32_t rc = grow_scratch(h, plan, npix, spp, accumulate == nullptr)) return rc;
+    const bool uses_lists = plan.tile_list_bytes != 0 && spp > 0 && !plan.halves &&
+                            (plan.kernel == RTX_KERNEL_WAVEFRONT || (plan.kernel == RTX_KERNEL_BVH && plan.spheres_two_stage));
+    RtxSceneHandle_::TileListKey key;
+    key.valid = true; key.scene_gen = h->scene_gen; key.cam = h->cam;
+    key.width = width; key.height = height; key.row_begin = row_begin; key.row_stride = row_stride; key.row_block = row_block;
+    key.n_rows = n_rows; key.tiles_x = plan.tiles_x;
+    key.kernel = plan.kernel; key.tuning = h->cfg.tuning;
+    key.buffer = h->tile_lists; key.bytes = (size_t)plan.tile_list_bytes;
+    const bool lists_current = RTX_TILE_LIST_REUSE != 0 && uses_lists && !h->sv_dirty && tile_list_key_equal(h->tl_key, key);
+    h->tl_key.valid = false;
 
     RowsView rv = rows_view(h, width, height, row_begin, row_stride, row_block, n_rows, plan.tiles_x, (uint32_t)plan.per_sample64);
     rv.nonzero = spp > 0 ? reinterpret_cast<uint32_t *>(h->samples + (size_t)(plan.batch * plan.per_sample64) * 4) : nullptr;
@@ -867,7 +902,8 @@
     } else if (plan.halves) {
         if (int32_t rc = launch_halves(h, plan, rv, d_out_rgb, stream, stats != nullptr, run)) return rc;
     } else {
-        if (int32_t rc = launch_batches(h, plan, rv, sr, d_out_rgb, stream, stats != nullptr, run)) return rc;
+        if (int32_t rc = launch_batches(h, plan, rv, sr, d_out_rgb, stream, stats != nullptr, run, lists_current)) return rc;
+        if (uses_lists) h->tl_key = key;
     }
     return finish_stats(h, plan, run, (uint64_t)npix * spp, stream, stats);
 }
diff --git a/rust-raytracing_amd/csrc/rtx_api_debug.hip b/rust-raytracing_amd/csrc/rtx_api_debug.hip
--- a/rust-raytracing_amd/csrc/rtx_api_debug.hip
+++ b/rust-raytracing_amd/csrc/rtx_api_debug.hip
@@ -566,7 +566,7 @@
     const size_t bytes = form == 1u ? bvh_spheres_tile_list_bytes((uint64_t)n_tiles << 6) : wavefront_tile_list_bytes((uint64_t)n_tiles << 6);
     const uint32_t cap = form == 0u ? 0u : (uint32_t)((form == 1u ? bvh_spheres_tile_list_bytes(64) - 256 : wavefront_tile_list_bytes(64) - 256) / entry_bytes);
     const uint32_t words = (uint32_t)(entry_bytes / sizeof(uint32_t));
-    const uint32_t head_info[8] = { form, h->tl_tiles_x, n_tiles, cap, words, 0u, 0u, 0u };
+    const uint32_t head_info[8] = { form, h->tl_tiles_x, n_tiles, cap, words, h->tl_builds, 0u, 0u };
     std::memcpy(info, head_info, sizeof head_info);
     if (form == 0u || n_tiles == 0u || (!counts && !entries)) return RTX_OK;
     if (!counts || !entries || max_tiles < n_tiles) return fail(RTX_ERR_INVALID_ARGUMENT, "rtx_debug_tile_lists: counts and entries hold info[2] tiles");
diff --git a/rust-raytracing_amd/csrc/rtx_api_update.hip b/rust-raytracing_amd/csrc/rtx_api_update.hip
--- a/rust-raytracing_amd/csrc/rtx_api_update.hip
+++ b/rust-raytracing_amd/csrc/rtx_api_update.hip
@@ -48,6 +48,7 @@
 int32_t apply_plan(RtxSceneHandle_ *h, UpdatePlan &plan, hipStream_t stream)
 {
     auto &b = h->upd;
+    touch_scene(h);
     if (int32_t rc = ensure_update_tables(h)) return rc;
     if (plan.tri_geom) if (int32_t rc = ensure_mesh_tables(h)) return rc;
     const RefitTables &t = h->refit;
@@ -132,6 +133,7 @@
 {
     if (!scene || (n_objects && !objects)) return fail(RTX_ERR_INVALID_ARGUMENT, "rtx_scene_append_objects: null argument");
     if (n_objects == 0) return RTX_OK;
+    touch_scene(scene);
     if (scene->objects.size() + n_objects > 0xFFFFFFF0ull) return fail(RTX_ERR_INVALID_ARGUMENT, "rtx_scene_append_objects: too many objects");
     RTX_HIP_CHECK(hipSetDevice(scene->device));
     RTX_HIP_CHECK(hipDeviceSynchronize());
@@ -147,6 +149,7 @@
 {
     if (how) *how = RTX_UPDATED_NOTHING;
     if (!h) return fail(RTX_ERR_INVALID_ARGUMENT, "rtx_scene_update_objects: null scene");
+    touch_scene(h);
     UpdatePlan plan;
     if (int32_t rc = plan_update(h->objects, h->refit, h->sv.sphere_cmax, indices, objects, n, mode, plan, h->hidden.empty() ? nullptr : h->hidden.data()))
         return rc;
@@ -174,6 +177,7 @@
 {
     if (how) *how = RTX_UPDATED_NOTHING;
     if (!h) return fail(RTX_ERR_INVALID_ARGUMENT, "rtx_scene_set_visible: null scene");
+    touch_scene(h);
     std::vector<uint8_t> hidden = hidden_bytes(h, h->objects.size());
     UpdatePlan plan;
     if (int32_t rc = plan_visibility(h->objects, hidden, h->refit, h->sv.sphere_cmax, indices, n, visible, plan)) return rc;
diff --git a/rust-raytracing_amd/csrc/rtx_bvh_spheres.hip b/rust-raytracing_amd/csrc/rtx_bvh_spheres.hip
--- a/rust-raytracing_amd/csrc/rtx_bvh_spheres.hip
+++ b/rust-raytracing_amd/csrc/rtx_bvh_spheres.hip
@@ -1,4 +1,5 @@
 #include "rtx_launch.h"
+#include "rtx_spk_pool.h"
 #include "rtx_spk_units.h"
 #include "rtx_traverse.h"
 
@@ -348,9 +349,58 @@
 #ifndef RTX_SPK_UNITS
 #define RTX_SPK_UNITS 1
 #endif
+#ifndef RTX_SPK_POOL
+#define RTX_SPK_POOL 1
+#endif
+#ifndef RTX_SPK_POOL_COUNT
+#define RTX_SPK_POOL_COUNT 0
+#endif
 #ifdef RTX_LAB
 constexpr uint32_t kSphNoPackets = 1u;
 #endif
+
+constexpr int kSpkPoolRows = 5;
+__device__ __forceinline__ void spk_pool_push(double2 *pw, uint32_t slot, const RayState &r, const Hit &h, uint32_t ridx)
+{
+    pw[0 * kBvhThreads + slot] = make_double2(r.pos.x, r.pos.y);
+    pw[1 * kBvhThreads + slot] = make_double2(r.pos.z, r.dir.x);
+    pw[2 * kBvhThreads + slot] = make_double2(r.dir.y, r.dir.z);
+    pw[3 * kBvhThreads + slot] = make_double2(__longlong_as_double((long long)r.key), h.t);
+    pw[4 * kBvhThreads + slot] = make_double2(__longlong_as_double(((long long)h.kind << 32) | (long long)h.id),
+                                              __longlong_as_double(((long long)ridx << 32) | (long long)h.local));
+    __builtin_amdgcn_fence(__ATOMIC_RELEASE, "wavefront");
+}
+
+__device__ __forceinline__ void spk_pool_pull(const double2 *pw, uint32_t slot, RayState &r, Hit &h, uint32_t &ridx)
+{
+    __builtin_amdgcn_fence(__ATOMIC_ACQUIRE, "wavefront");
+    const double2 a = pw[0 * kBvhThreads + slot], b = pw[1 * kBvhThreads + slot], c = pw[2 * kBvhThreads + slot],
+                  d = pw[3 * kBvhThreads + slot], e = pw[4 * kBvhThreads + slot];
+    r.pos = mk(a.x, a.y, b.x);
+    r.dir = mk(b.y, c.x, c.y);
+    r.result = mk(0., 0., 0.); r.light = mk(1., 1., 1.); r.draw = 6; r.bounce = 0;
+    r.key = (uint64_t)__double_as_longlong(d.x);
+    h.t = d.y;
+    const uint64_t ik = (uint64_t)__double_as_longlong(e.x), lr = (uint64_t)__double_as_longlong(e.y);
+    h.id = (uint32_t)ik; h.kind = (uint32_t)(ik >> 32);
+    h.local = (uint32_t)lr; ridx = (uint32_t)(lr >> 32);
+}
+
+__device__ __forceinline__ void spk_shade_hits(const SceneView &sv, const RowsView &rv, double *__restrict__ samples, const SphQueue &sq,
+                                               Counters *__restrict__ ctr, bool have, RayState &r, const Hit &h, uint32_t ridx,
+                                               uint32_t bounce_limit, uint32_t lane, unsigned long long &out_next, unsigned long long &out_end)
+{
+    uint32_t first_id = 0;
+    bool go = false;
+    if (have) {
+        advance_and_shade<kRoundGlobal>(sv, h, r);
+        first_id = h.id;
+        const bool done = (r.bounce >= bounce_limit) || light_is_zero(r);
+        if (done) store_sample<kRoundGlobal>(samples, rv, ridx, r.result);
+        go = !done;
+    }
+    sph_queue_append(sq, ctr, go, r, ridx, first_id, lane, out_next, out_end);
+}
 
 
 
@@ -504,6 +554,14 @@
 #endif
     unsigned long long out_next = 0, out_end = 0;
     unsigned long long segs = 0, box_tests = 0, leaf_filters = 0, exact = 0;
+#if RTX_SPK_POOL
+    __shared__ double2 lds_pool[kSpkPoolRows][kBvhThreads];
+    double2 *const pw = &lds_pool[0][0] + (tid & ~63u);
+    uint32_t pool = 0;
+#if RTX_SPK_POOL_COUNT
+    unsigned long long shade_passes = 0;
+#endif
+#endif
 
 #ifndef RTX_SPK_GRAB_MUL
 #define RTX_SPK_GRAB_MUL 2
@@ -634,10 +692,16 @@
                 }
 #undef RTX_SPK_WALK
             }
+#if RTX_SPK_POOL
+            Hit h;
+            hit_init(h);
+            if (alive) {
+#else
             uint32_t first_id = 0;
             if (alive) {
                 Hit h;
                 hit_init(h);
+#endif
                 ++segs;
                 box_tests += nbox;
                 leaf_filters += nleaf;
@@ -668,6 +732,22 @@
                     if (triangle_distance(la.tris[tk], rx, &t)) hit_consider(h, t, la.tris[tk].id, 2, tk);
                 }
                 exact += sv.n_planes + sv.n_tri_filter;
+#if RTX_SPK_POOL
+            }
+            const unsigned long long hm = __ballot(alive && h.id != kNone);
+            const SpkPoolStep ps = spk_pool_lane(hm, lane, pool);
+            if (spk_pool_shades(hm, pool)) {
+                uint32_t hridx = ridx;
+                if (ps.action == kSpkPoolPull) spk_pool_pull(pw, ps.slot, r, h, hridx);
+                spk_shade_hits(sv, rv, samples, sq, ctr, true, r, h, hridx, bounce_limit, lane, out_next, out_end);
+#if RTX_SPK_POOL_COUNT
+                ++shade_passes;
+#endif
+            } else if (ps.action == kSpkPoolPush) {
+                spk_pool_push(pw, ps.slot, r, h, ridx);
+            }
+            pool = spk_pool_next(hm, pool);
+#else
 
                 bool done = true;
                 if (h.id != kNone) {
@@ -681,8 +761,27 @@
                 }
             }
             sph_queue_append(sq, ctr, alive, r, ridx, first_id, lane, out_next, out_end);
-        }
-    }
+#endif
+        }
+    }
+#if RTX_SPK_POOL
+    if (pool != 0u) {
+        const SpkPoolStep ps = spk_pool_flush_lane(lane, pool);
+        RayState r;
+        Hit h;
+        uint32_t hridx = 0;
+        hit_init(h);
+        r.pos = mk(0., 0., 0.); r.dir = mk(1., 0., 0.); r.result = mk(0., 0., 0.); r.light = mk(1., 1., 1.); r.key = 0; r.draw = 6; r.bounce = 0;
+        if (ps.action == kSpkPoolPull) spk_pool_pull(pw, ps.slot, r, h, hridx);
+        spk_shade_hits(sv, rv, samples, sq, ctr, ps.action == kSpkPoolPull, r, h, hridx, bounce_limit, lane, out_next, out_end);
+#if RTX_SPK_POOL_COUNT
+        ++shade_passes;
+#endif
+    }
+#if RTX_SPK_POOL_COUNT
+    if (lane == 0 && shade_passes) atomicAdd(&ctr[0].pad_, shade_passes);
+#endif
+#endif
     sph_queue_close(sq, lane, out_next, out_end);
     unsigned long long filt = box_tests + leaf_filters;
 #pragma unroll
diff --git a/rust-raytracing_amd/csrc/rtx_host.h b/rust-raytracing_amd/csrc/rtx_host.h
--- a/rust-raytracing_amd/csrc/rtx_host.h
+++ b/rust-raytracing_amd/csrc/rtx_host.h
@@ -42,8 +42,17 @@
     double *state = nullptr;    size_t state_bytes = 0;
     void *wf_state = nullptr;   size_t wf_bytes = 0;
     void *tile_lists = nullptr; size_t tile_lists_bytes = 0;
+    uint64_t scene_gen = 0;
+    struct TileListKey {
+        bool valid = false;
+        uint64_t scene_gen = 0;
+        RtxCamera cam{};
+        uint32_t width = 0, height = 0, row_begin = 0, row_stride = 0, row_block = 0, n_rows = 0, tiles_x = 0;
+        uint32_t kernel = 0, tuning = 0;
+        const void *buffer = nullptr; size_t bytes = 0;
+    } tl_key;
 #ifdef RTX_LAB
-    uint32_t tl_form = 0, tl_tiles_x = 0, tl_tiles = 0;
+    uint32_t tl_form = 0, tl_tiles_x = 0, tl_tiles = 0, tl_builds = 0;
 #endif
     PathStep *transcript = nullptr; uint32_t *transcript_counts = nullptr; uint32_t transcript_steps = 0;
     Counters *counters = nullptr;
@@ -76,6 +85,8 @@
 
 RTX_HOST_BEGIN
 
+inline void touch_scene(RtxSceneHandle_ *h) { ++h->scene_gen; h->tl_key.valid = false; }
+
 inline size_t nonzero_mask_bytes(uint64_t n_rays) { return (size_t)((n_rays + 31) / 32) * sizeof(uint32_t); }
 
 struct SampleRange { uint64_t begin = 0, n = 0; double *sum = nullptr, *sum_sq = nullptr; };
diff --git a/rust-raytracing_amd/csrc/rtx_spk_pool.h b/rust-raytracing_amd/csrc/rtx_spk_pool.h
--- /dev/null
+++ b/rust-raytracing_amd/csrc/rtx_spk_pool.h
@@ -0,0 +1,61 @@
+#pragma once
+
+#include <stdint.h>
+
+#if defined(__HIPCC__) || defined(__CUDACC__)
+#define RTX_SPK_POOL_HD __host__ __device__ inline
+#else
+#define RTX_SPK_POOL_HD inline
+#endif
+
+namespace rtx {
+
+constexpr uint32_t kSpkPoolSlots = 64;
+
+enum SpkPoolAction : uint32_t {
+    kSpkPoolKeep = 0,
+    kSpkPoolPush = 1,
+    kSpkPoolPull = 2,
+    kSpkPoolIdle = 3
+};
+
+struct SpkPoolStep { uint32_t action, slot; };
+
+RTX_SPK_POOL_HD uint32_t spk_pool_popcount(uint64_t m)
+{
+    return (uint32_t)__builtin_popcountll((unsigned long long)m);
+}
+
+RTX_SPK_POOL_HD bool spk_pool_shades(uint64_t m, uint32_t pool) { return pool + spk_pool_popcount(m) >= kSpkPoolSlots; }
+
+RTX_SPK_POOL_HD uint32_t spk_pool_next(uint64_t m, uint32_t pool)
+{
+    const uint32_t n = spk_pool_popcount(m);
+    return pool + n >= kSpkPoolSlots ? pool + n - kSpkPoolSlots : pool + n;
+}
+
+RTX_SPK_POOL_HD SpkPoolStep spk_pool_lane(uint64_t m, uint32_t lane, uint32_t pool)
+{
+    const bool hit = ((m >> lane) & 1ull) != 0ull;
+    const uint32_t hits_below = spk_pool_popcount(m & ((1ull << lane) - 1ull));
+    const uint32_t idle_below = lane - hits_below;
+    SpkPoolStep s;
+    if (spk_pool_shades(m, pool)) {
+        s.action = hit ? kSpkPoolKeep : kSpkPoolPull;
+        s.slot = hit ? 0u : pool - 1u - idle_below;
+    } else {
+        s.action = hit ? kSpkPoolPush : kSpkPoolIdle;
+        s.slot = hit ? pool + hits_below : 0u;
+    }
+    return s;
+}
+
+RTX_SPK_POOL_HD SpkPoolStep spk_pool_flush_lane(uint32_t lane, uint32_t pool)
+{
+    SpkPoolStep s;
+    s.action = lane < pool ? kSpkPoolPull : kSpkPoolIdle;
+    s.slot = lane < pool ? lane : 0u;
+    return s;
+}
+
+}
```

New measurement: 4319 Mrays/s (median of 6 runs). 1.6% higher.
